# LiWentomng/OrientedRepPoints

Measured on NVIDIA H100. Metric: 1024x1024 tiles/sec, higher is better.
Workload: dtype f16x3

## Files before the change

include/orp_b200.h:

```cpp
#ifndef ORP_B200_H_
#define ORP_B200_H_

#include <stdint.h>

#ifdef __cplusplus
extern "C" {
#endif

#define ORP_OK 0
#define ORP_EINVAL (-1)
#define ORP_ECUDA (-2)
#define ORP_ENOGPU (-3)
#define ORP_EOVERFLOW (-4)

const char *orp_last_error(void);
int orp_version(void);
int orp_compiled_sm(void);
int64_t orp_launch_count(void);
void orp_reset_launch_count(void);


#define ORP_NMS_EXACT64 0
#define ORP_NMS_COMPAT32 1

#define ORP_UNION_NAN_KEEPS 0
#define ORP_UNION_GUARD 1
#define ORP_UNION_NAN_SUPPRESSES 2
#define ORP_UNION_NAN_SUPPRESSES_ALL 3

#define ORP_ORDER_INDEX_ASC 0
#define ORP_ORDER_SCORE_DESC 1

int orp_rnms(const float *dets, const int32_t *segments, int n, double iou_thr, int iou_mode,
             int union_mode, int order, int64_t *keep_out, int32_t *num_out, void *stream);

int orp_poly_nms_host(int *keep_out, int *num_out, const float *polys_host, int polys_num,
                      int polys_dim, float nms_overlap_thresh, int device_id);

typedef struct {
    int64_t pairs_total;
    int64_t pairs_aabb;
    int64_t pairs_clipped;
    int64_t pairs_fp64;
    int64_t edges;
    int64_t suppressing;
    int32_t overflow;
    int32_t rounds;
    int32_t n;
} orp_nms_stats;
int orp_rnms_last_stats(orp_nms_stats *out);

typedef struct {
    int32_t lazy;
    int32_t R;
    int32_t seg_limit;
    int32_t sweep_bits;
    int32_t no_sync;
    int32_t flags_out;
    int32_t union_mode, order, n;
    int64_t cap_first;
    int64_t cap_final;
    int32_t attempts;
} orp_rnms_plan;
int orp_rnms_last_plan(orp_rnms_plan *out);

void orp_set_timing(int on);
int orp_rnms_last_sweep_ms(float *ms);
int orp_tc_timing_collect(float *total_ms, int *launches, double *flops);
typedef struct {
    int BN;
    int stages;
    int grid;
    int num_tiles;
    int n_tiles_n;
    int ksplit;
    int nprob;
    int Cout, Cout_padded;
    int split;
    int deform;
    int out_f32;
    int stem;
    int relu;
    int bias;
    int residual;
    int tma_epi, ncat, dcat, res_mma, b_resident, epi_merge, epi_bufs, gn_fused;
    int BW[5], BH[5], BI[5];
    int n_pair;
} orp_tc_plan;
int orp_tc_last_plan(orp_tc_plan *out);


int orp_poly_overlaps_host(float *overlaps, const float *boxes, const float *query_boxes, int n,
                           int k, int device_id);
int orp_poly_overlaps(const float *boxes5, int n, const float *query5, int k, float *out,
                      void *stream);

int orp_quad_iou_matrix(const float *quads_a, int n, const float *quads_b, int k, int iou_mode,
                        int union_mode, float *out, void *stream);

int orp_iou_poly_f64_pairs(const double *p8, const double *q8, int n, double *out, void *stream);

int orp_convex_iou(const float *pts18, int n, const float *quads8, int k, float *out, void *stream);

int orp_box_iou_rotated(const float *boxes1, int n, const float *boxes2, int m, float *out,
                        void *stream);


int orp_minarearect(const float *pts, int n, float *out, int32_t *hull_map, float scale,
                    const float *center, void *stream);


int orp_head_postprocess(int nlevels, const float *const *cls, const float *const *ref, const int *H,
                         const int *W, const int *stride, int B, int num_cls, int nms_pre, float score_thr,
                         double iou_thr, int max_per_img, const float *scale_factor, float *dets_out,
                         int64_t *labels_out, int32_t *counts_out, void *stream);
int orp_head_postprocess_aug(int nviews, int nlevels, const float *const *cls, const float *const *ref, const int *H,
                             const int *W, const int *stride, int B, int num_cls, int nms_pre, float score_thr,
                             double iou_thr, int max_per_img, const float *view_meta, const float *out_scale,
                             float *dets_out, int64_t *labels_out, int32_t *counts_out, void *stream);
int orp_pack_detections(const float *dets, const int64_t *labels, const int32_t *counts, int B, int max_per_img,
                        float *packed_out, void *stream);
int orp_dcn_offsets_multi(int nprob, const float *const *pts, float *const *off, const long long *numel,
                          float gradient_mul, const float *base18, void *stream);


#define ORP_MERGE_BAD_COUNT 1
#define ORP_MERGE_BAD_TILE 2
#define ORP_MERGE_ROWS_OVERFLOW 4

int orp_result_merge(const float *packed, int S, int cap, const int32_t *tile_slot, const int32_t *tile_xy,
                     const double *tile_rate, const int32_t *tile_img, int Tn, int ncls, int nimg, double thresh,
                     int union_mode, int max_rows, int32_t *count_out, int64_t *cls_off_out, int32_t *cls_out,
                     int32_t *img_out, double *score_out, double *quad_out, int32_t *src_row_out, int32_t *status_out,
                     void *stream);


int orp_dota_eval_task1(const int32_t *det_cls, const int32_t *det_img, const double *det_score, const double *det_quad,
                        int nd, const int32_t *gt_cls, const int32_t *gt_img, const double *gt_quad,
                        const uint8_t *gt_difficult, int ng, int ncls, int nimg, double ovthresh, int use_07_metric,
                        const double *thresholds11, int64_t *npos_out, int64_t *cls_off_out, int32_t *order_out,
                        double *rec_out, double *prec_out, double *ap_out, void *stream);

int orp_poly2rbox_v3(const double *quad, int n, double *out, void *stream);

int orp_dota_eval_aoe(const int32_t *det_cls, const int32_t *det_img, const double *det_score, const double *det_quad,
                      int nd, const int32_t *gt_cls, const int32_t *gt_img, const double *gt_quad, int ng, int ncls,
                      int nimg, double ovthresh, int64_t *cls_off_out, int32_t *order_out, double *angle_dif_out,
                      int64_t *count_out, double *aoe_out, void *stream);


int orp_convex_giou(const float *pts18, const float *quads8, int n, float *out19, void *stream);


int orp_conv2d_f32(const float *x, int N, int H, int W, int Cin, const float *w, int Cout, int KH, int KW,
                   int stride, int pad, const float *bias, const float *residual, int relu, float *y,
                   double *gn_stats, int groups, void *stream);

int orp_deform_conv2d_f32(const float *x, int N, int H, int W, int Cin, const float *offset, const float *mask,
                          const float *w, int Cout, int KH, int KW, int stride, int pad, int dilation,
                          const float *bias, int relu, float *y, void *stream);

int orp_gn_apply_f32(const float *x, int N, int H, int W, int C, const double *stats, int groups,
                     const float *gamma, const float *beta, float eps, int relu, const float *up_src, float *y,
                     void *stream);

int orp_maxpool3x3s2_f32(const float *x, int N, int H, int W, int C, float *y, void *stream);


typedef struct {
    const void *x;
    int N, H, W;
    void *out;
    const void *residual_bf16;
    const float *residual_f32;
    const float *offset;
    double *gn_stats;
    const float *mask;
} orp_tc_problem;

int orp_conv2d_bf16(int nprob, const orp_tc_problem *probs, const void *w, int Cout, int Cout_padded,
                    int KH, int KW, int Cin, int stride, int pad, const float *bias, int relu, int out_f32,
                    int deform, void *stream);

int orp_conv2d_f16x3(int nprob, const orp_tc_problem *probs, const void *w_split, int Cout, int Cout_padded,
                     int KH, int KW, int Cin, int stride, int pad, const float *bias, int wscale_log2, int relu,
                     int out_f32, int deform, void *stream);
int orp_conv2d_tc_splitk(const orp_tc_problem *prob, const void *w, int Cout, int Cout_padded, int KH, int KW, int Cin,
                         int stride, int pad, const float *bias, int f16x3, int wscale_log2, int relu, int ksplit,
                         float *workspace, void *stream);
int orp_tc_plan_conv(int nprob, const orp_tc_problem *probs, const void *w, int Cout, int Cout_padded, int KH, int KW,
                     int Cin, int stride, int pad, const float *bias, int wscale_log2, int relu, int out_f32, int deform,
                     int split, int stem, int ksplit, int sms, orp_tc_plan *out);
int orp_f16x3_overflow_count(unsigned int *count, int reset, void *stream);
int orp_stem_s2d_u8_f16x3(const uint8_t *img_hwc, int N, int H, int W, const float *mean, const float *std, int to_rgb,
                          void *out, void *stream);
int orp_stem_s2d_u8_padded_f16x3(const uint8_t *img_hwc, int N, int H, int W, const float *mean, const float *std, int to_rgb,
                                 const int32_t *valid_hw, void *out, void *stream);
int orp_stem_s2d_f16x3(const float *img_nchw, int N, int H, int W, void *out, void *stream);
int orp_stem_conv_s2d_f16x3(const void *x_s2d, int N, int H, int W, const void *w_split, const float *bias,
                            int wscale_log2, int relu, void *out, void *stream);
int orp_maxpool3x3s2_f16x3(const void *x, int N, int H, int W, int C, void *y, void *stream);
int orp_gn_stats_f16x3(const void *x, int N, int HW, int C, int groups, double *stats, void *stream);
int orp_split_from_f32(const float *x, long long pixels, int C, void *y_split, void *stream);
int orp_split_to_f32(const void *x_split, long long pixels, int C, float *y, void *stream);
int orp_transpose_f32(const float *x, int N, int R, int Cc, float *y, void *stream);
int orp_nchw_f32_to_split(const float *x, int N, int C, int HW, void *y_split, void *stream);

int orp_stem_im2col_bf16(const float *img_nchw, int N, int H, int W, void *out, void *stream);
int orp_stem_s2d_bf16(const float *img_nchw, int N, int H, int W, void *out, void *stream);
int orp_stem_conv_s2d_bf16(const void *x_s2d, int N, int H, int W, const void *w256, const float *bias, int relu,
                           void *out, void *stream);
int orp_stem_s2d_u8_bf16(const uint8_t *img_hwc, int N, int H, int W, const float *mean, const float *std, int to_rgb,
                         void *out, void *stream);
int orp_stem_s2d_u8_padded_bf16(const uint8_t *img_hwc, int N, int H, int W, const float *mean, const float *std, int to_rgb,
                                const int32_t *valid_hw, void *out, void *stream);
int orp_maxpool3x3s2_bf16(const void *x, int N, int H, int W, int C, void *y, void *stream);
int orp_gn_stats_bf16(const void *x, int N, int HW, int C, int groups, double *stats, void *stream);
typedef struct orp_gn_problem {
    const void *x;
    int N, H, W;
    const double *stats;
    const void *up_src;
    void *y;
} orp_gn_problem;
int orp_gn_apply_bf16_multi(int nprob, const orp_gn_problem *probs, int C, int groups, const float *gamma,
                            const float *beta, float eps, int relu, void *stream);
int orp_gn_apply_f16x3_multi(int nprob, const orp_gn_problem *probs, int C, int groups, const float *gamma,
                             const float *beta, float eps, int relu, void *stream);

int orp_split_tiles_u8(const uint8_t *img_hwc, int H, int W, int C, const int32_t *origins, int ntiles, int subsize,
                       uint8_t *out, void *stream);

int orp_resize_u8(const uint8_t *src, int N, int H, int W, int C, uint8_t *dst, int Hd, int Wd, int Hp, int Wp, int flip,
                  const int32_t *xtab, const int32_t *ytab, void *stream);


int orp_layernorm_bf16(const void *x, int B, int H, int W, int C, const float *gamma, const float *beta, float eps,
                       int Hp, int Wp, void *y, void *stream);
int orp_window_attention_bf16(const void *qkv, int B, int H, int W, int Hp, int Wp, int C, int heads, int shift,
                              const float *bias_table, float scale, void *out, void *stream);
int orp_patch_embed_rows_bf16(const float *img_nchw, int B, int H, int W, void *out, void *stream);
int orp_patch_embed_rows_u8_bf16(const uint8_t *img_hwc, int B, int H, int W, const float *mean, const float *stdinv, int to_rgb,
                                 void *out, void *stream);
int orp_patch_embed_rows_u8_padded_bf16(const uint8_t *img_hwc, int B, int H, int W, const float *mean, const float *stdinv,
                                        int to_rgb, const int32_t *valid_hw, void *out, void *stream);
int orp_patch_merge_gather_bf16(const void *x, int B, int H, int W, int C, void *y, void *stream);
int orp_subsample2_bf16(const void *x, int B, int H, int W, int C, void *y, void *stream);
int orp_layernorm_f16x3(const void *x, int B, int H, int W, int C, const float *gamma, const float *beta, float eps,
                        int Hp, int Wp, void *y, void *stream);
int orp_window_attention_f16x3(const void *qkv, int B, int H, int W, int Hp, int Wp, int C, int heads, int shift,
                               const float *bias_table, float scale, void *out, void *stream);
int orp_patch_embed_rows_f16x3(const float *img_nchw, int B, int H, int W, void *out, void *stream);
int orp_patch_embed_rows_u8_f16x3(const uint8_t *img_hwc, int B, int H, int W, const float *mean, const float *stdinv, int to_rgb,
                                  void *out, void *stream);
int orp_patch_embed_rows_u8_padded_f16x3(const uint8_t *img_hwc, int B, int H, int W, const float *mean, const float *stdinv,
                                         int to_rgb, const int32_t *valid_hw, void *out, void *stream);
int orp_patch_merge_gather_f16x3(const void *x, int B, int H, int W, int C, void *y, void *stream);
int orp_subsample2_f16x3(const void *x, int B, int H, int W, int C, void *y, void *stream);

#ifdef __cplusplus
}
#endif
#endif
```

orientedreppoints_b200/_lib.py:

```python
import ctypes
import os

_HERE = os.path.dirname(os.path.abspath(__file__))
LIB_PATH = os.path.join(_HERE, "lib", "liborp_b200.so")

ORP_NMS_EXACT64, ORP_NMS_COMPAT32 = 0, 1
ORP_UNION_NAN_KEEPS, ORP_UNION_GUARD, ORP_UNION_NAN_SUPPRESSES, ORP_UNION_NAN_SUPPRESSES_ALL = 0, 1, 2, 3
ORP_ORDER_INDEX_ASC, ORP_ORDER_SCORE_DESC = 0, 1
ORP_MERGE_BAD_COUNT, ORP_MERGE_BAD_TILE, ORP_MERGE_ROWS_OVERFLOW = 1, 2, 4

_vp = ctypes.c_void_p
_i = ctypes.c_int
_f = ctypes.c_float
_d = ctypes.c_double


class NmsStats(ctypes.Structure):
    _fields_ = [("pairs_total", ctypes.c_int64), ("pairs_aabb", ctypes.c_int64),
                ("pairs_clipped", ctypes.c_int64), ("pairs_fp64", ctypes.c_int64),
                ("edges", ctypes.c_int64), ("suppressing", ctypes.c_int64), ("overflow", ctypes.c_int32),
                ("rounds", ctypes.c_int32), ("n", ctypes.c_int32)]

    def as_dict(self):
        return {k: int(getattr(self, k)) for k, _ in self._fields_}


class RnmsPlan(ctypes.Structure):
    _fields_ = [(k, ctypes.c_int32) for k in ("lazy", "R", "seg_limit", "sweep_bits", "no_sync", "flags_out", "union_mode",
                                              "order", "n")] + \
              [("cap_first", ctypes.c_int64), ("cap_final", ctypes.c_int64), ("attempts", ctypes.c_int32)]

    def as_dict(self):
        return {k: int(getattr(self, k)) for k, _ in self._fields_}


class TcProblem(ctypes.Structure):
    _fields_ = [("x", _vp), ("N", _i), ("H", _i), ("W", _i), ("out", _vp), ("residual_bf16", _vp),
                ("residual_f32", _vp), ("offset", _vp), ("gn_stats", _vp), ("mask", _vp)]


class TcPlan(ctypes.Structure):
    _fields_ = [(k, _i) for k in ("BN", "stages", "grid", "num_tiles", "n_tiles_n", "ksplit", "nprob", "Cout", "Cout_padded",
                                  "split", "deform", "out_f32", "stem", "relu", "bias", "residual", "tma_epi", "ncat", "dcat",
                                  "res_mma", "b_resident", "epi_merge", "epi_bufs", "gn_fused")] + \
              [(k, _i * 5) for k in ("BW", "BH", "BI")] + [("n_pair", _i)]

    def as_dict(self):
        d = {k: getattr(self, k) for k, _ in self._fields_}
        for k in ("BW", "BH", "BI"):
            d[k] = list(d[k])[:self.nprob]
        return d


class GnProblem(ctypes.Structure):
    _fields_ = [("x", _vp), ("N", _i), ("H", _i), ("W", _i), ("stats", _vp), ("up_src", _vp), ("y", _vp)]


SIGNATURES = {
    "orp_last_error": (ctypes.c_char_p, []),
    "orp_version": (_i, []),
    "orp_compiled_sm": (_i, []),
    "orp_launch_count": (ctypes.c_int64, []),
    "orp_reset_launch_count": (None, []),
    "orp_rnms": (_i, [_vp, _vp, _i, _d, _i, _i, _i, _vp, _vp, _vp]),
    "orp_poly_nms_host": (_i, [_vp, _vp, _vp, _i, _i, _f, _i]),
    "orp_rnms_last_stats": (_i, [ctypes.POINTER(NmsStats)]),
    "orp_rnms_last_plan": (_i, [ctypes.POINTER(RnmsPlan)]),
    "orp_set_timing": (None, [_i]),
    "orp_rnms_last_sweep_ms": (_i, [ctypes.POINTER(ctypes.c_float)]),
    "orp_tc_timing_collect": (_i, [ctypes.POINTER(ctypes.c_float), ctypes.POINTER(_i), ctypes.POINTER(_d)]),
    "orp_tc_last_plan": (_i, [ctypes.POINTER(TcPlan)]),
    "orp_poly_overlaps_host": (_i, [_vp, _vp, _vp, _i, _i, _i]),
    "orp_poly_overlaps": (_i, [_vp, _i, _vp, _i, _vp, _vp]),
    "orp_quad_iou_matrix": (_i, [_vp, _i, _vp, _i, _i, _i, _vp, _vp]),
    "orp_iou_poly_f64_pairs": (_i, [_vp, _vp, _i, _vp, _vp]),
    "orp_box_iou_rotated": (_i, [_vp, _i, _vp, _i, _vp, _vp]),
    "orp_minarearect": (_i, [_vp, _i, _vp, _vp, _f, _vp, _vp]),
    "orp_head_postprocess": (_i, [_i, _vp, _vp, _vp, _vp, _vp, _i, _i, _i, _f, _d, _i, _vp, _vp, _vp, _vp, _vp]),
    "orp_head_postprocess_aug": (_i, [_i, _i, _vp, _vp, _vp, _vp, _vp, _i, _i, _i, _f, _d, _i, _vp, _vp, _vp, _vp, _vp, _vp]),
    "orp_pack_detections": (_i, [_vp, _vp, _vp, _i, _i, _vp, _vp]),
    "orp_dcn_offsets_multi": (_i, [_i, _vp, _vp, _vp, _f, _vp, _vp]),
    "orp_conv2d_f32": (_i, [_vp, _i, _i, _i, _i, _vp, _i, _i, _i, _i, _i, _vp, _vp, _i, _vp, _vp, _i, _vp]),
    "orp_deform_conv2d_f32": (_i, [_vp, _i, _i, _i, _i, _vp, _vp, _vp, _i, _i, _i, _i, _i, _i, _vp, _i, _vp, _vp]),
    "orp_gn_apply_f32": (_i, [_vp, _i, _i, _i, _i, _vp, _i, _vp, _vp, _f, _i, _vp, _vp, _vp]),
    "orp_maxpool3x3s2_f32": (_i, [_vp, _i, _i, _i, _i, _vp, _vp]),
    "orp_conv2d_bf16": (_i, [_i, ctypes.POINTER(TcProblem), _vp, _i, _i, _i, _i, _i, _i, _i, _vp, _i, _i, _i, _vp]),
    "orp_conv2d_f16x3": (_i, [_i, ctypes.POINTER(TcProblem), _vp, _i, _i, _i, _i, _i, _i, _i, _vp, _i, _i, _i, _i, _vp]),
    "orp_conv2d_tc_splitk": (_i, [ctypes.POINTER(TcProblem), _vp, _i, _i, _i, _i, _i, _i, _i, _vp, _i, _i, _i, _i, _vp, _vp]),
    "orp_tc_plan_conv": (_i, [_i, ctypes.POINTER(TcProblem), _vp, _i, _i, _i, _i, _i, _i, _i, _vp, _i, _i, _i, _i, _i, _i, _i, _i,
                              ctypes.POINTER(TcPlan)]),
    "orp_f16x3_overflow_count": (_i, [ctypes.POINTER(ctypes.c_uint), _i, _vp]),
    "orp_stem_s2d_u8_f16x3": (_i, [_vp, _i, _i, _i, _vp, _vp, _i, _vp, _vp]),
    "orp_stem_s2d_f16x3": (_i, [_vp, _i, _i, _i, _vp, _vp]),
    "orp_stem_conv_s2d_f16x3": (_i, [_vp, _i, _i, _i, _vp, _vp, _i, _i, _vp, _vp]),
    "orp_maxpool3x3s2_f16x3": (_i, [_vp, _i, _i, _i, _i, _vp, _vp]),
    "orp_gn_stats_f16x3": (_i, [_vp, _i, _i, _i, _i, _vp, _vp]),
    "orp_gn_apply_f16x3_multi": (_i, [_i, _vp, _i, _i, _vp, _vp, _f, _i, _vp]),
    "orp_split_from_f32": (_i, [_vp, ctypes.c_longlong, _i, _vp, _vp]),
    "orp_split_to_f32": (_i, [_vp, ctypes.c_longlong, _i, _vp, _vp]),
    "orp_transpose_f32": (_i, [_vp, _i, _i, _i, _vp, _vp]),
    "orp_nchw_f32_to_split": (_i, [_vp, _i, _i, _i, _vp, _vp]),
    "orp_layernorm_bf16": (_i, [_vp, _i, _i, _i, _i, _vp, _vp, _f, _i, _i, _vp, _vp]),
    "orp_window_attention_bf16": (_i, [_vp, _i, _i, _i, _i, _i, _i, _i, _i, _vp, _f, _vp, _vp]),
    "orp_patch_embed_rows_bf16": (_i, [_vp, _i, _i, _i, _vp, _vp]),
    "orp_patch_embed_rows_u8_bf16": (_i, [_vp, _i, _i, _i, _vp, _vp, _i, _vp, _vp]),
    "orp_patch_merge_gather_bf16": (_i, [_vp, _i, _i, _i, _i, _vp, _vp]),
    "orp_subsample2_bf16": (_i, [_vp, _i, _i, _i, _i, _vp, _vp]),
    "orp_layernorm_f16x3": (_i, [_vp, _i, _i, _i, _i, _vp, _vp, _f, _i, _i, _vp, _vp]),
    "orp_window_attention_f16x3": (_i, [_vp, _i, _i, _i, _i, _i, _i, _i, _i, _vp, _f, _vp, _vp]),
    "orp_patch_embed_rows_f16x3": (_i, [_vp, _i, _i, _i, _vp, _vp]),
    "orp_patch_embed_rows_u8_f16x3": (_i, [_vp, _i, _i, _i, _vp, _vp, _i, _vp, _vp]),
    "orp_patch_merge_gather_f16x3": (_i, [_vp, _i, _i, _i, _i, _vp, _vp]),
    "orp_subsample2_f16x3": (_i, [_vp, _i, _i, _i, _i, _vp, _vp]),
    "orp_stem_im2col_bf16": (_i, [_vp, _i, _i, _i, _vp, _vp]),
    "orp_stem_s2d_bf16": (_i, [_vp, _i, _i, _i, _vp, _vp]),
    "orp_convex_iou": (_i, [_vp, _i, _vp, _i, _vp, _vp]),
    "orp_convex_giou": (_i, [_vp, _vp, _i, _vp, _vp]),
    "orp_dota_eval_task1": (_i, [_vp, _vp, _vp, _vp, _i, _vp, _vp, _vp, _vp, _i, _i, _i, _d, _i, _vp, _vp, _vp, _vp, _vp,
                                 _vp, _vp, _vp]),
    "orp_dota_eval_aoe": (_i, [_vp, _vp, _vp, _vp, _i, _vp, _vp, _vp, _i, _i, _i, _d, _vp, _vp, _vp, _vp, _vp, _vp]),
    "orp_poly2rbox_v3": (_i, [_vp, _i, _vp, _vp]),
    "orp_result_merge": (_i, [_vp, _i, _i, _vp, _vp, _vp, _vp, _i, _i, _i, _d, _i, _i, _vp, _vp, _vp, _vp, _vp, _vp, _vp, _vp,
                              _vp]),
    "orp_split_tiles_u8": (_i, [_vp, _i, _i, _i, _vp, _i, _i, _vp, _vp]),
    "orp_resize_u8": (_i, [_vp, _i, _i, _i, _i, _vp, _i, _i, _i, _i, _i, _vp, _vp, _vp]),
    "orp_stem_s2d_u8_padded_bf16": (_i, [_vp, _i, _i, _i, _vp, _vp, _i, _vp, _vp, _vp]),
    "orp_stem_s2d_u8_padded_f16x3": (_i, [_vp, _i, _i, _i, _vp, _vp, _i, _vp, _vp, _vp]),
    "orp_patch_embed_rows_u8_padded_bf16": (_i, [_vp, _i, _i, _i, _vp, _vp, _i, _vp, _vp, _vp]),
    "orp_patch_embed_rows_u8_padded_f16x3": (_i, [_vp, _i, _i, _i, _vp, _vp, _i, _vp, _vp, _vp]),
    "orp_stem_s2d_u8_bf16": (_i, [_vp, _i, _i, _i, _vp, _vp, _i, _vp, _vp]),
    "orp_stem_conv_s2d_bf16": (_i, [_vp, _i, _i, _i, _vp, _vp, _i, _vp, _vp]),
    "orp_maxpool3x3s2_bf16": (_i, [_vp, _i, _i, _i, _i, _vp, _vp]),
    "orp_gn_stats_bf16": (_i, [_vp, _i, _i, _i, _i, _vp, _vp]),
    "orp_gn_apply_bf16_multi": (_i, [_i, _vp, _i, _i, _vp, _vp, _f, _i, _vp]),
}

_LIB = None


class OrpError(RuntimeError):
    pass


def lib():
    global _LIB
    if _LIB is None:
        if not os.path.exists(LIB_PATH):
            raise OrpError(
                "liborp_b200.so not found at %s - build it with `python -m orientedreppoints_b200.build` "
                "(there is no CPU or PyTorch fallback for this path)" % LIB_PATH)
        l = ctypes.CDLL(LIB_PATH)
        for name, (res, args) in SIGNATURES.items():
            fn = getattr(l, name)
            fn.restype = res
            fn.argtypes = args
        _LIB = l
    return _LIB


def check(rc, what=""):
    if rc != 0:
        msg = lib().orp_last_error()
        raise OrpError("%s failed (%d): %s" % (what, rc, msg.decode() if msg else ""))


def launch_count():
    return int(lib().orp_launch_count())


def reset_launch_count():
    lib().orp_reset_launch_count()


def last_nms_stats():
    s = NmsStats()
    check(lib().orp_rnms_last_stats(ctypes.byref(s)), "orp_rnms_last_stats")
    return s.as_dict()


def rnms_last_plan():
    p = RnmsPlan()
    check(lib().orp_rnms_last_plan(ctypes.byref(p)), "orp_rnms_last_plan")
    return p.as_dict()


def set_timing(on):
    lib().orp_set_timing(1 if on else 0)


def last_sweep_ms():
    v = ctypes.c_float(0)
    check(lib().orp_rnms_last_sweep_ms(ctypes.byref(v)), "orp_rnms_last_sweep_ms")
    return float(v.value)


def tc_timing_collect():
    ms, n, fl = ctypes.c_float(0), ctypes.c_int(0), ctypes.c_double(0)
    check(lib().orp_tc_timing_collect(ctypes.byref(ms), ctypes.byref(n), ctypes.byref(fl)), "orp_tc_timing_collect")
    return float(ms.value), int(n.value), float(fl.value)


def tc_last_plan():
    p = TcPlan()
    check(lib().orp_tc_last_plan(ctypes.byref(p)), "orp_tc_last_plan")
    return p.as_dict()


def tc_plan_for(problems, cout, cout_p, kh, kw, cin, stride, pad, *, bias=False, relu=0, out_f32=False, deform=False,
                split=False, residual=0, gn=False, stem=0, ksplit=1, sms=132):
    ph = 256
    arr = (TcProblem * len(problems))()
    for q, (n, h, w) in zip(arr, problems):
        q.x, q.N, q.H, q.W, q.out = ph, n, h, w, ph
        q.residual_bf16 = ph if residual == 1 else None
        q.residual_f32 = ph if residual == 2 else None
        q.offset = ph if deform else None
        q.gn_stats = ph if gn else None
    p = TcPlan()
    check(lib().orp_tc_plan_conv(len(problems), arr, ph, cout, cout_p, kh, kw, cin, stride, pad, ph if bias else None, 0,
                                 int(relu), int(out_f32), int(deform), int(split), stem, ksplit, sms, ctypes.byref(p)),
          "orp_tc_plan_conv")
    return p.as_dict()


def current_stream_ptr():
    import torch
    return ctypes.c_void_p(torch.cuda.current_stream().cuda_stream)


def ptr(t):
    return ctypes.c_void_p(0 if t is None else t.data_ptr())
```

orientedreppoints_b200/csrc/dense_tc.cu:

```cuda
#include <cuda.h>
#include <cuda_bf16.h>
#include <cuda_fp16.h>

#include <cstdlib>
#include <mutex>
#include <type_traits>

#include "common.cuh"
#include "wgmma.cuh"

namespace orp {
namespace {

constexpr int kMaxProb = 5;
constexpr int kStagesMax = 6;
constexpr int kBM = 128;
constexpr int kBK = 64;
constexpr int kABytes = kBM * kBK * 2;

struct FastDiv {
    uint32_t mul, shr, d;
    __host__ void set(uint32_t div)
    {
        d = div;
        uint32_t l = 0;
        while ((1ull << l) < div) ++l;
        shr = l;
        mul = (uint32_t)(((1ull << 32) * ((1ull << l) - div)) / div + 1);
    }
    __device__ __forceinline__ uint32_t div(uint32_t n) const { return (__umulhi(n, mul) + n) >> shr; }
    __device__ __forceinline__ void divmod(uint32_t n, uint32_t &q, uint32_t &r) const { q = div(n); r = n - q * d; }
};

struct Problem {
    int N, H, W, Ho, Wo;
    FastDiv fd_tw, fd_th;
    int BW, BH, BI;
    int lbw, lbh;
    int tiles_w, tiles_h, tiles_i, tile_start;
    void *out;
    const __nv_bfloat16 *res;
    const float *res32;
    const __nv_bfloat16 *x;
    const float *offset;
    const float *mask;
    double *gn_stats;
};

struct alignas(64) TcParams {
    CUtensorMap tmA[kMaxProb];
    CUtensorMap tmB;
    CUtensorMap tmOut[kMaxProb];
    CUtensorMap tmRes[kMaxProb];
    CUtensorMap tmI;
    Problem prob[kMaxProb];
    int tma_epi, epi_bufs;
    int epi_merge;
    int ncat;
    int ksplit;
    FastDiv fd_ks;
    long long ks_stride;
    int b_resident;
    int res_mma;
    int gn_fused;
    int dcat;
    int split;
    float oscale;
    unsigned int *ovf;
    int nprob, num_m_tiles, n_tiles_n, num_tiles;
    FastDiv fd_ntn;
    int KH, KW, Cin, cin_blocks, stride, pad, Cout, relu;
    int s2d_stem;
    const float *bias;
};

__device__ __forceinline__ uint32_t smem_u32(const void *p) { return (uint32_t)__cvta_generic_to_shared(p); }

__device__ __forceinline__ void mbar_init(uint64_t *bar, uint32_t count)
{
    asm volatile("mbarrier.init.shared::cta.b64 [%0], %1;" ::"r"(smem_u32(bar)), "r"(count));
}
__device__ __forceinline__ void mbar_expect_tx(uint64_t *bar, uint32_t bytes)
{
    asm volatile("mbarrier.arrive.expect_tx.shared::cta.b64 _, [%0], %1;" ::"r"(smem_u32(bar)), "r"(bytes) : "memory");
}
__device__ __forceinline__ void mbar_arrive(uint64_t *bar)
{
    asm volatile("mbarrier.arrive.shared::cta.b64 _, [%0];" ::"r"(smem_u32(bar)) : "memory");
}
__device__ __forceinline__ void mbar_wait(uint64_t *bar, uint32_t parity)
{
    asm volatile(
        "{\n\t"
        ".reg .pred p;\n\t"
        "WAIT_LOOP:\n\t"
        "mbarrier.try_wait.parity.shared::cta.b64 p, [%0], %1;\n\t"
        "@p bra WAIT_DONE;\n\t"
        "bra WAIT_LOOP;\n\t"
        "WAIT_DONE:\n\t"
        "}" ::"r"(smem_u32(bar)), "r"(parity) : "memory");
}
__device__ __forceinline__ bool elect_one()
{
    uint32_t pred = 0;
    asm volatile(
        "{\n\t"
        ".reg .pred P1;\n\t"
        "elect.sync _|P1, %1;\n\t"
        "selp.b32 %0, 1, 0, P1;\n\t"
        "}" : "=r"(pred) : "r"(0xffffffffu));
    return pred != 0;
}
__device__ __forceinline__ void tma_load_4d(void *smem, const CUtensorMap *tm, uint64_t *bar, int c0, int c1, int c2, int c3)
{
    asm volatile(
        "cp.async.bulk.tensor.4d.shared::cluster.global.mbarrier::complete_tx::bytes [%0], [%1, {%3, %4, %5, %6}], [%2];"
        ::"r"(smem_u32(smem)), "l"(tm), "r"(smem_u32(bar)), "r"(c0), "r"(c1), "r"(c2), "r"(c3) : "memory");
}
__device__ __forceinline__ void tma_load_5d(void *smem, const CUtensorMap *tm, uint64_t *bar, int c0, int c1, int c2, int c3, int c4)
{
    asm volatile(
        "cp.async.bulk.tensor.5d.shared::cluster.global.mbarrier::complete_tx::bytes [%0], [%1, {%3, %4, %5, %6, %7}], [%2];"
        ::"r"(smem_u32(smem)), "l"(tm), "r"(smem_u32(bar)), "r"(c0), "r"(c1), "r"(c2), "r"(c3), "r"(c4) : "memory");
}
__device__ __forceinline__ void tma_load_2d(void *smem, const CUtensorMap *tm, uint64_t *bar, int c0, int c1)
{
    asm volatile(
        "cp.async.bulk.tensor.2d.shared::cluster.global.mbarrier::complete_tx::bytes [%0], [%1, {%3, %4}], [%2];"
        ::"r"(smem_u32(smem)), "l"(tm), "r"(smem_u32(bar)), "r"(c0), "r"(c1) : "memory");
}
__device__ __forceinline__ uint64_t make_desc_sw128(uint32_t smem_addr)
{
    uint64_t d = 0;
    d |= (uint64_t)((smem_addr >> 4) & 0x3FFF);
    d |= (uint64_t)1 << 16;
    d |= (uint64_t)(1024 >> 4) << 32;
    d |= (uint64_t)1 << 62;
    return d;
}
__device__ __forceinline__ uint4 lds128(uint32_t addr)
{
    uint4 v;
    asm volatile("ld.shared.v4.b32 {%0, %1, %2, %3}, [%4];" : "=r"(v.x), "=r"(v.y), "=r"(v.z), "=r"(v.w) : "r"(addr) : "memory");
    return v;
}
__device__ __forceinline__ void sts128(uint32_t addr, const uint4 &v)
{
    asm volatile("st.shared.v4.b32 [%0], {%1, %2, %3, %4};" ::"r"(addr), "r"(v.x), "r"(v.y), "r"(v.z), "r"(v.w) : "memory");
}
template <int ID, int N>
__device__ __forceinline__ void named_bar()
{
    asm volatile("bar.sync %0, %1;" ::"n"(ID), "n"(N) : "memory");
}
__device__ __forceinline__ void acc_ld32(uint32_t addr, uint32_t (&r)[32])
{
#pragma unroll
    for (int j = 0; j < 8; ++j) {
        const uint4 v = lds128(addr + (uint32_t)j * 16u);
        r[4 * j] = v.x; r[4 * j + 1] = v.y; r[4 * j + 2] = v.z; r[4 * j + 3] = v.w;
    }
}

__device__ __forceinline__ float2 ffma2_rn(float2 a, float2 b, float2 c) { return make_float2(__fmaf_rn(a.x, b.x, c.x), __fmaf_rn(a.y, b.y, c.y)); }
__device__ __forceinline__ float2 fadd2_rn(float2 a, float2 b) { return make_float2(__fadd_rn(a.x, b.x), __fadd_rn(a.y, b.y)); }

__device__ __forceinline__ void split_sample(const uint4 (&u)[4][2], float4 wv, uint2 wh, uint32_t (&hi)[4], uint32_t (&lo)[4])
{
    const float2 wc[4] = {make_float2(wv.x, wv.x), make_float2(wv.y, wv.y), make_float2(wv.z, wv.z), make_float2(wv.w, wv.w)};
    const __half2 wl[4] = {__low2half2(*reinterpret_cast<const __half2 *>(&wh.x)), __high2half2(*reinterpret_cast<const __half2 *>(&wh.x)),
                           __low2half2(*reinterpret_cast<const __half2 *>(&wh.y)), __high2half2(*reinterpret_cast<const __half2 *>(&wh.y))};
#pragma unroll
    for (int k = 0; k < 4; ++k) {
        float2 acc = make_float2(0.f, 0.f);
        __half2 accl = __float2half2_rn(0.f);
#pragma unroll
        for (int c = 0; c < 4; ++c) {
            const uint32_t uh = reinterpret_cast<const uint32_t *>(&u[c][0])[k];
            const uint32_t ul = reinterpret_cast<const uint32_t *>(&u[c][1])[k];
            acc = ffma2_rn(wc[c], __half22float2(*reinterpret_cast<const __half2 *>(&uh)), acc);
            accl = __hfma2(wl[c], *reinterpret_cast<const __half2 *>(&ul), accl);
        }
        acc = fadd2_rn(acc, __half22float2(accl));
        const __half2 h2 = __floats2half2_rn(acc.x, acc.y);
        const float2 hf = __half22float2(h2);
        const float2 rem = fadd2_rn(acc, make_float2(-hf.x, -hf.y));
        const __half2 l2 = __floats2half2_rn(rem.x, rem.y);
        hi[k] = *reinterpret_cast<const uint32_t *>(&h2);
        lo[k] = *reinterpret_cast<const uint32_t *>(&l2);
    }
}

__device__ __forceinline__ float act_fn(float v, int act)
{
    if (act == 1) return fmaxf(v, 0.f);
    if (act == 2) return 0.5f * v * (1.0f + erff(v * 0.70710678118654752f));
    return v;
}

struct Ring {
    int stage = 0;
    uint32_t phase = 0;
    int n;
    __device__ explicit Ring(int n_) : n(n_) {}
    __device__ void next() { if (++stage == n) { stage = 0; phase ^= 1; } }
};

struct KIter {
    int tap, term, cb = 0, phase = 0;
    int tap0, taps, cbn, mode;
    __device__ KIter(int taps_, int cbn_, int mode_, int tap0_ = 0) : tap0(tap0_), taps(taps_), cbn(cbn_), mode(mode_)
    {
        tap = tap0;
        term = (mode == 1) ? 1 : 0;
    }
    __device__ void next()
    {
        if (mode == 0) { if (++cb == cbn) { cb = 0; ++tap; } }
        else if (phase == 0) {
            if (++cb == cbn) { cb = 0; if (++term == 3) { term = 1; if (++tap == taps) { tap = tap0; term = 0; phase = 1; } } }
        } else { if (++cb == cbn) { cb = 0; ++tap; } }
    }
};

__device__ __forceinline__ int ksplit_of(const TcParams &P, int tile)
{
    if (P.ksplit <= 1) return 0;
    uint32_t q, r;
    P.fd_ks.divmod((uint32_t)tile, q, r);
    return (int)r;
}

__device__ __forceinline__ void decode_tile(const TcParams &P, int tile, int &pi, int &wb, int &hb, int &ib, int &nt)
{
    uint32_t mt_u, nt_u;
    if (P.ksplit > 1) tile = (int)P.fd_ks.div((uint32_t)tile);
    P.fd_ntn.divmod((uint32_t)tile, mt_u, nt_u);
    nt = (int)nt_u;
    const int mt = (int)mt_u;
    pi = 0;
#pragma unroll
    for (int k = 1; k < kMaxProb; ++k)
        if (k < P.nprob && mt >= P.prob[k].tile_start) pi = k;
    const Problem &pr = P.prob[pi];
    const int local = mt - pr.tile_start;
    uint32_t rest, wb_u, ib_u, hb_u;
    pr.fd_tw.divmod((uint32_t)local, rest, wb_u);
    pr.fd_th.divmod(rest, ib_u, hb_u);
    wb = (int)wb_u; hb = (int)hb_u; ib = (int)ib_u;
}

struct IdentBlock { unsigned short v[64 * 64]; };
constexpr IdentBlock make_ident()
{
    IdentBlock b{};
    for (int i = 0; i < 64; ++i) b.v[i * 64 + i] = 0x3F80;
    return b;
}
__device__ IdentBlock g_ident = make_ident();
struct IdentBlocks16 { unsigned short v[16][64 * 64]; };
constexpr IdentBlocks16 make_ident16()
{
    IdentBlocks16 b{};
    for (int s = 0; s < 16; ++s)
        for (int i = 0; i < 64; ++i) b.v[s][i * 64 + i] = (unsigned short)((15 + s) << 10);
    return b;
}
__device__ IdentBlocks16 g_ident16 = make_ident16();
__device__ unsigned int g_f16_overflow = 0;

constexpr int kConsumers = 256;
constexpr int kDP = 256;
constexpr int kDItems = 1024 / kDP;
constexpr int kDRound = kDItems / 2;
constexpr int kAccPitch = 68;
constexpr int kAccBytes = 128 * kAccPitch * 4;

__host__ __device__ constexpr int stage_bytes(int BN, bool cat, bool b_resident)
{
    return cat ? (b_resident ? 2 * kABytes : 2 * kABytes + 2 * BN * kBK * 2) : (b_resident ? kABytes : kABytes + BN * kBK * 2);
}
__host__ __device__ constexpr bool frag_epilogue(int BN, bool deform) { return deform && BN == 256; }
constexpr int dyn_smem_bytes(int stage_b, int stages, int extra, bool frag_epi)
{
    return 1024 + (frag_epi ? 0 : kAccBytes) + stages * stage_b + extra;
}

template <int BN, int R>
__device__ __forceinline__ void stage_acc(const float (&acc)[R], int pass, bool ncat, float *s_acc, int row0, int col0)
{
    constexpr int kGroups = (BN < 64 ? BN : 64) / 8;
#pragma unroll
    for (int p = 0; p < (BN + 63) / 64; ++p) {
        if (p != pass) continue;
#pragma unroll
        for (int i = 0; i < kGroups; ++i) {
            const int g = p * 8 + i;
            float2 a = make_float2(acc[4 * g], acc[4 * g + 1]), b = make_float2(acc[4 * g + 2], acc[4 * g + 3]);
            if constexpr (R >= BN) {
                if (ncat) {
                    a.x += acc[BN / 2 + 4 * g]; a.y += acc[BN / 2 + 4 * g + 1];
                    b.x += acc[BN / 2 + 4 * g + 2]; b.y += acc[BN / 2 + 4 * g + 3];
                }
            }
            *reinterpret_cast<float2 *>(s_acc + row0 * kAccPitch + i * 8 + col0) = a;
            *reinterpret_cast<float2 *>(s_acc + (row0 + 8) * kAccPitch + i * 8 + col0) = b;
        }
    }
}

constexpr int kWalkK = 0;
constexpr int kWalkNcat = 1;
constexpr int kWalkDcat = 2;
constexpr int kWalkKRes = 3;

template <int NG, bool BF16, int R, int G = 0>
__device__ __forceinline__ void wgmma_cols64(float (&acc)[R], uint64_t da, uint64_t db, uint32_t accumulate)
{
    wgmma_n<64, BF16>(acc_view<32 * G, 32>(acc), da, db + (uint64_t)(G * 512), accumulate);
    if constexpr (G + 1 < NG) wgmma_cols64<NG, BF16, R, G + 1>(acc, da, db, accumulate);
}

template <int BN, bool BF16>
__device__ __forceinline__ void wgmma_dcat(float (&acc)[BN / 2], uint64_t da, uint64_t db, uint32_t accumulate)
{
    if constexpr (BN == 256) {
        wgmma_n<128, BF16>(acc_view<0, 64>(acc), da, db, accumulate);
        wgmma_n<128, BF16>(acc_view<64, 64>(acc), da, db + (uint64_t)1024, accumulate);
    } else {
        wgmma_n<BN, BF16>(acc, da, db, accumulate);
    }
}

constexpr int kProducerRegs = 40;
constexpr int kConsumerRegs = 232;
constexpr int kWideConsumerRegs = 160;
constexpr int kWideProducerRegs = 96;

template <int BN, bool OUT_F32, bool DEFORM, bool SPLIT, int WALK>
__global__ void __launch_bounds__(DEFORM ? kConsumers + kDP : kConsumers + 128, 1)
conv_tc_kernel(const __grid_constant__ TcParams P, int stages)
{
    static_assert(WALK != kWalkNcat || (SPLIT && !DEFORM && !OUT_F32 && BN >= 64 && BN <= 128), "ncat: f16x3 TMA-epilogue layers, BN 64..128");
    static_assert(!DEFORM || (WALK == kWalkDcat) == SPLIT, "deformable: dcat exactly in f16x3");
    static_assert(DEFORM || WALK != kWalkDcat, "dcat is the deformable walk");
    static_assert(WALK != kWalkKRes || (!DEFORM && !OUT_F32 && BN >= 64), "residual K blocks: TMA-epilogue layers");
    constexpr bool kBF16 = !SPLIT;
    constexpr int kWTerms = SPLIT ? 2 : 1;
    constexpr bool kCat = WALK == kWalkNcat || WALK == kWalkDcat;
    constexpr int kKMode = (SPLIT && !kCat) ? 1 : 0;
    static_assert(kConsumers + 128 == 384 && 2 * 128 * kConsumerRegs + 128 * kProducerRegs <= 65536, "register split");
    constexpr bool kFragEpi = frag_epilogue(BN, DEFORM);
    static_assert(!kFragEpi || (SPLIT && !OUT_F32), "fragment epilogue: deformable f16x3 with a TMA epilogue");
    static_assert(kConsumers == 256 && kDP == 256 && 2 * 128 * kWideConsumerRegs + 2 * 128 * kWideProducerRegs <= 65536,
                  "register split (wide deformable)");
    constexpr int kEpiThreads = kConsumers;
    constexpr int kWG = 2;
    constexpr int kAccN = (WALK == kWalkNcat) ? 2 * BN : BN;
    extern __shared__ __align__(1024) uint8_t smem_raw[];
    uint8_t *smem = reinterpret_cast<uint8_t *>((reinterpret_cast<uintptr_t>(smem_raw) + 1023) & ~uintptr_t(1023));
    float *s_acc = reinterpret_cast<float *>(smem);
    if constexpr (!kFragEpi) smem += kAccBytes;
    constexpr int kBBytes = BN * kBK * 2;
    const int kStageBytes = stage_bytes(BN, kCat, P.b_resident);
    const int kblocks_all = P.KH * P.KW * P.cin_blocks * kWTerms;
    uint8_t *ident = smem;
    if (P.res_mma) smem += 8192;
    uint8_t *bres = smem;
    if (P.b_resident) smem += (size_t)kblocks_all * kBBytes;
    constexpr int HC = BN < 64 ? BN : 64;
    constexpr int kPitch = HC * 2 + 16;
    uint8_t *stage_out = smem + (size_t)stages * kStageBytes;
    __shared__ uint64_t bars[2 * kStagesMax];
    __shared__ __align__(16) float s_bias[256];
    __shared__ uint64_t bres_bar;
    uint64_t *full = bars;
    uint64_t *empty = bars + kStagesMax;

    const int warp = threadIdx.x >> 5, lane = threadIdx.x & 31;

    if (warp == kConsumers / 32 && elect_one()) {
        if (!DEFORM) {
#pragma unroll 1
            for (int p = 0; p < P.nprob; ++p)
                asm volatile("prefetch.tensormap [%0];" ::"l"(&P.tmA[p]) : "memory");
        }
        asm volatile("prefetch.tensormap [%0];" ::"l"(&P.tmB) : "memory");
    }
    if (warp == 0) {
        if (elect_one()) {
            for (int s = 0; s < stages; ++s) {
                mbar_init(&full[s], DEFORM ? 1 + kDP / 32 : 1);
                mbar_init(&empty[s], kConsumers / 128);
            }
            mbar_init(&bres_bar, 1);
            asm volatile("fence.mbarrier_init.release.cluster;" ::: "memory");
        }
        __syncwarp();
    }
    __syncthreads();
    const int taps_per = (P.KH * P.KW) / (P.ksplit > 1 ? P.ksplit : 1);
    const int kblocks = taps_per * P.cin_blocks * (kKMode ? 3 : 1);
    asm volatile("griddepcontrol.launch_dependents;" ::: "memory");
    asm volatile("griddepcontrol.wait;" ::: "memory");

    if (warp < kConsumers / 32) {
        if constexpr (!DEFORM) setmaxnreg_inc<kConsumerRegs>();
        if constexpr (kFragEpi) setmaxnreg_inc<kWideConsumerRegs>();
        const int cw = warp >> 2;
        const uint32_t a_off = (uint32_t)cw * 8192u;
        const bool leader = (threadIdx.x & 127) == 0;
        float acc[kAccN / 2];
        Ring r(stages);
        const int q = warp & 3, wg = warp >> 2;
        const int et = threadIdx.x, nthr = kEpiThreads;
        const int bar_a = 1, bar_b = 3;
        const int ch0 = wg, chs = kWG;
        const int frow = cw * 64 + (warp & 3) * 16 + (lane >> 2), fcol = 2 * (lane & 3);
        const uint32_t s_acc_u = smem_u32(s_acc);
        auto bar_sync = [](int id, int n) { asm volatile("bar.sync %0, %1;" ::"r"(id), "r"(n) : "memory"); };
        int ob = 0;
        int bias_nt = -1;
        if ((P.b_resident || P.res_mma) && (int)blockIdx.x < P.num_tiles) mbar_wait(&bres_bar, 0);
        for (int tile = blockIdx.x; tile < P.num_tiles; tile += gridDim.x) {
            int res_groups = 0;
            if constexpr (WALK == kWalkKRes) {
                const int nt = tile - (int)P.fd_ntn.div((uint32_t)tile) * P.n_tiles_n;
                for (int g = 0; g < BN / 64 && nt * BN + g * 64 < P.Cout; ++g) ++res_groups;
            }
            const int tap_lo = ksplit_of(P, tile) * taps_per;
            KIter it(tap_lo + taps_per, P.cin_blocks, kKMode, tap_lo);
            int held = -1;
            auto release = [&](int next) {
                if (held >= 0 && leader) mbar_arrive(&empty[held]);
                held = next;
            };
            for (int kb = 0; kb < kblocks; ++kb, it.next()) {
                if constexpr (kFragEpi) {
                    wgmma_wait<0>();
                    release(-1);
                }
                mbar_wait(&full[r.stage], r.phase);
                const uint32_t sa = smem_u32(smem + (size_t)r.stage * kStageBytes);
                const uint64_t da = make_desc_sw128(sa + a_off);
                const int slab = (it.tap * P.cin_blocks + it.cb) * kWTerms + (it.term == 2 ? 1 : 0);
                wgmma_fence();
                if constexpr (WALK == kWalkNcat) {
                    const uint32_t sb = P.b_resident ? smem_u32(bres + (size_t)slab * kBBytes) : sa + 2 * kABytes;
                    const uint64_t dl = make_desc_sw128(sa + kABytes + a_off);
                    const uint64_t dbh = make_desc_sw128(sb), dbl = make_desc_sw128(sb + kBBytes);
#pragma unroll
                    for (int k = 0; k < kBK / 16; ++k) {
                        const uint32_t first = (kb | k) ? 1u : 0u;
                        wgmma_n<BN, kBF16>(acc_view<0, BN / 2>(acc), da + (uint64_t)(k * 2), dbh + (uint64_t)(k * 2), first);
                        wgmma_n<BN, kBF16>(acc_view<BN / 2, BN / 2>(acc), da + (uint64_t)(k * 2), dbl + (uint64_t)(k * 2), first);
                        wgmma_n<BN, kBF16>(acc_view<BN / 2, BN / 2>(acc), dl + (uint64_t)(k * 2), dbh + (uint64_t)(k * 2), 1u);
                    }
                } else if constexpr (WALK == kWalkDcat) {
                    const uint64_t dl = make_desc_sw128(sa + kABytes + a_off);
                    const uint64_t dbh = make_desc_sw128(sa + 2 * kABytes), dbl = make_desc_sw128(sa + 2 * kABytes + kBBytes);
#pragma unroll
                    for (int k = 0; k < kBK / 16; ++k) {
                        wgmma_dcat<BN, kBF16>(acc, dl + (uint64_t)(k * 2), dbh + (uint64_t)(k * 2), (kb | k) ? 1u : 0u);
                        wgmma_dcat<BN, kBF16>(acc, da + (uint64_t)(k * 2), dbl + (uint64_t)(k * 2), 1u);
                        wgmma_dcat<BN, kBF16>(acc, da + (uint64_t)(k * 2), dbh + (uint64_t)(k * 2), 1u);
                    }
                } else {
                    const uint64_t db = make_desc_sw128(P.b_resident ? smem_u32(bres + (size_t)slab * kBBytes) : sa + kABytes);
#pragma unroll
                    for (int k = 0; k < kBK / 16; ++k) {
                        if constexpr (WALK == kWalkKRes)
                            wgmma_cols64<BN / 64, kBF16>(acc, da + (uint64_t)(k * 2), db + (uint64_t)(k * 2), (kb | k) ? 1u : 0u);
                        else
                            wgmma_n<BN, kBF16>(acc, da + (uint64_t)(k * 2), db + (uint64_t)(k * 2), (kb | k) ? 1u : 0u);
                    }
                }
                wgmma_commit();
                wgmma_wait<1>();
                release(r.stage);
                r.next();
            }
            if constexpr (WALK == kWalkKRes) {
                wgmma_wait<0>();
                release(-1);
                auto res_group = [&](auto gc) {
                    constexpr int G = decltype(gc)::value;
                    if (G >= res_groups) return;
#pragma unroll 1
                    for (int t = 0; t < kWTerms; ++t) {
                        mbar_wait(&full[r.stage], r.phase);
                        const uint64_t da = make_desc_sw128(smem_u32(smem + (size_t)r.stage * kStageBytes) + a_off);
                        const uint64_t db = make_desc_sw128(smem_u32(ident));
                        wgmma_fence();
#pragma unroll
                        for (int k = 0; k < kBK / 16; ++k)
                            wgmma_n<64, kBF16>(acc_view<32 * G, 32>(acc), da + (uint64_t)(k * 2), db + (uint64_t)(k * 2), 1u);
                        wgmma_commit();
                        wgmma_wait<1>();
                        release(r.stage);
                        r.next();
                    }
                };
                res_group(std::integral_constant<int, 0>{});
                if constexpr (BN >= 128) res_group(std::integral_constant<int, 1>{});
                if constexpr (BN >= 256) {
                    res_group(std::integral_constant<int, 2>{});
                    res_group(std::integral_constant<int, 3>{});
                }
            }
            wgmma_wait<0>();
            wgmma_fence_acc(acc);
            release(-1);

            int pi, wb, hb, ib, nt;
            decode_tile(P, tile, pi, wb, hb, ib, nt);
            const Problem &pr = P.prob[pi];
            const int rrow = q * 32 + lane;
            auto row_pixel = [&](int r, size_t &pix) -> bool {
                const int iw = r & (pr.BW - 1), ih = (r >> pr.lbw) & (pr.BH - 1), ii = r >> (pr.lbw + pr.lbh);
                const int w = wb * pr.BW + iw, h = hb * pr.BH + ih, n = ib * pr.BI + ii;
                pix = ((size_t)n * pr.Ho + h) * pr.Wo + w;
                return (w < pr.Wo) && (h < pr.Ho) && (n < pr.N);
            };
            size_t pix;
            const bool valid = row_pixel(rrow, pix);
            if constexpr (kFragEpi) {
                const uint32_t obuf_u = smem_u32(stage_out);
                const bool io = (et == 0);
                if (nt != bias_nt) {
                    bar_sync(bar_a, nthr);
                    for (int c = et; c < BN; c += nthr) s_bias[c] = (P.bias && nt * BN + c < P.Cout) ? P.bias[nt * BN + c] : 0.f;
                    bias_nt = nt;
                }
                size_t pix_r[2];
                const bool valid_r[2] = {row_pixel(frow, pix_r[0]), row_pixel(frow + 8, pix_r[1])};
                float amax[2][2] = {{0.f, 0.f}, {0.f, 0.f}};
#pragma unroll
                for (int pass = 0; pass < 2 * (BN / 64); ++pass) {
                    const int half = pass >> 1, oterm = pass & 1;
                    if (io) {
                        if (P.epi_bufs == 2) asm volatile("cp.async.bulk.wait_group.read 1;" ::: "memory");
                        else asm volatile("cp.async.bulk.wait_group.read 0;" ::: "memory");
                    }
                    bar_sync(bar_a, nthr);
                    const uint32_t obase = obuf_u + (uint32_t)ob * 16384u;
#pragma unroll
                    for (int i = 0; i < 8; ++i) {
                        const int g = half * 8 + i;
                        const float2 bv = *reinterpret_cast<const float2 *>(&s_bias[g * 8 + fcol]);
#pragma unroll
                        for (int hr = 0; hr < 2; ++hr) {
                            const int row = frow + 8 * hr;
                            float f0 = acc[4 * g + 2 * hr], f1 = acc[4 * g + 2 * hr + 1];
                            f0 *= P.oscale; f1 *= P.oscale;
                            f0 += bv.x; f1 += bv.y;
                            if (P.relu) { f0 = fmaxf(f0, 0.f); f1 = fmaxf(f1, 0.f); }
                            if (oterm == 0) amax[hr][i >> 2] = fmaxf(fmaxf(amax[hr][i >> 2], fabsf(f0)), fabsf(f1));
                            const __half2 h2 = __floats2half2_rn(f0, f1);
                            uint32_t v = *reinterpret_cast<const uint32_t *>(&h2);
                            if (oterm) {
                                const float2 hf = __half22float2(h2);
                                const __half2 l2 = __floats2half2_rn(f0 - hf.x, f1 - hf.y);
                                v = *reinterpret_cast<const uint32_t *>(&l2);
                            }
                            const uint32_t at = obase + (uint32_t)row * 128u + ((uint32_t)(i ^ (row & 7)) << 4) + (uint32_t)fcol * 2u;
                            asm volatile("st.shared.b32 [%0], %1;" ::"r"(at), "r"(v) : "memory");
                        }
                    }
                    asm volatile("fence.proxy.async.shared::cta;" ::: "memory");
                    bar_sync(bar_b, nthr);
                    if (io) {
                        asm volatile(
                            "cp.async.bulk.tensor.5d.global.shared::cta.bulk_group [%0, {%2, %3, %4, %5, %6}], [%1];"
                            ::"l"(&P.tmOut[pi]), "r"(obase), "r"(nt * BN + half * 64), "r"(oterm),
                              "r"(wb * pr.BW), "r"(hb * pr.BH), "r"(ib * pr.BI) : "memory");
                        asm volatile("cp.async.bulk.commit_group;" ::: "memory");
                    }
                    if (++ob == P.epi_bufs) ob = 0;
                }
#pragma unroll
                for (int hr = 0; hr < 2; ++hr)
#pragma unroll
                    for (int hc = 0; hc < 2; ++hc) {
                        float m = amax[hr][hc];
                        m = fmaxf(m, __shfl_xor_sync(0xffffffffu, m, 1));
                        m = fmaxf(m, __shfl_xor_sync(0xffffffffu, m, 2));
                        if ((lane & 3) == 0 && valid_r[hr] && m > 65504.f) atomicAdd(P.ovf, 1u);
                    }
            } else if (OUT_F32) {
#pragma unroll 1
                for (int pass = 0; pass < BN / HC; ++pass) {
                bar_sync(bar_a, nthr);
                stage_acc<BN>(acc, pass, false, s_acc, frow, fcol);
                bar_sync(bar_a, nthr);
#pragma unroll 1
                for (int ch = wg; ch < HC / 32; ch += kWG) {
                    uint32_t v[32];
                    acc_ld32(s_acc_u + (uint32_t)(rrow * kAccPitch + ch * 32) * 4u, v);
                    const int c0 = nt * BN + pass * HC + ch * 32;
                    if (valid && c0 < P.Cout) {
                        float *op = reinterpret_cast<float *>(pr.out) + pix * P.Cout + c0;
                        const float *rp = pr.res32 ? pr.res32 + pix * P.Cout + c0 : nullptr;
                        if (P.ksplit > 1) {
                            float *sp = op + (long long)ksplit_of(P, tile) * P.ks_stride;
                            for (int j = 0; j < 32; ++j) {
                                if (c0 + j >= P.Cout) break;
                                sp[j] = __uint_as_float(v[j]) * P.oscale;
                            }
                        } else
                        for (int j = 0; j < 32; ++j) {
                            if (c0 + j >= P.Cout) break;
                            float f = __uint_as_float(v[j]) * P.oscale;
                            if (P.bias) f += P.bias[c0 + j];
                            if (pr.res && !P.split) f += __bfloat162float(pr.res[pix * P.Cout + c0 + j]);
                            if (rp) f += rp[j];
                            f = act_fn(f, P.relu);
                            op[j] = f;
                        }
                    }
                }
                }
            } else if (P.tma_epi) {
                const uint32_t slot = P.epi_merge ? 32768u : 16384u;
                const uint32_t obuf_u = smem_u32(stage_out);
                const uint32_t bias_u = smem_u32(s_bias);
                const bool io = (et == 0);
                constexpr int kPasses = BN / 64;
                const int oterms = (P.split && !P.epi_merge) ? 2 : 1;
                if (nt != bias_nt) {
                    bar_sync(bar_a, nthr);
                    for (int c = et; c < BN; c += nthr) s_bias[c] = (P.bias && nt * BN + c < P.Cout) ? P.bias[nt * BN + c] : 0.f;
                    bias_nt = nt;
                }
                float amax = 0.f;
#pragma unroll 1
                for (int pass = 0; pass < kPasses * oterms; ++pass) {
                    const int half = oterms == 2 ? (pass >> 1) : pass, oterm = oterms == 2 ? (pass & 1) : 0;
                    if (io) {
                        if (P.epi_bufs == 2) asm volatile("cp.async.bulk.wait_group.read 1;" ::: "memory");
                        else asm volatile("cp.async.bulk.wait_group.read 0;" ::: "memory");
                    }
                    bar_sync(bar_a, nthr);
                    if (oterm == 0) {
                        stage_acc<BN>(acc, half, P.ncat != 0, s_acc, frow, fcol);
                        bar_sync(bar_a, nthr);
                    }
                    float gn_s = 0.f, gn_q = 0.f;
                    const uint32_t orow = obuf_u + (uint32_t)ob * slot + (uint32_t)rrow * 128u;
#pragma unroll 1
                    for (int ch = ch0; ch < 2; ch += chs) {
                        const uint32_t arow = s_acc_u + (uint32_t)(rrow * kAccPitch + ch * 32) * 4u;
#pragma unroll
                        for (int j4 = 0; j4 < 4; ++j4) {
                            const int c16 = ch * 4 + j4;
                            const uint32_t sw = (uint32_t)(c16 ^ (rrow & 7)) << 4;
                            const uint4 a0 = lds128(arow + (uint32_t)j4 * 32u), a1 = lds128(arow + (uint32_t)j4 * 32u + 16u);
                            const float f0[8] = {__uint_as_float(a0.x), __uint_as_float(a0.y), __uint_as_float(a0.z), __uint_as_float(a0.w),
                                                 __uint_as_float(a1.x), __uint_as_float(a1.y), __uint_as_float(a1.z), __uint_as_float(a1.w)};
                            float f[8];
#pragma unroll
                            for (int j = 0; j < 8; ++j) f[j] = f0[j];
                            const uint32_t bb = bias_u + (uint32_t)(half * 64 + ch * 32 + j4 * 8) * 4u;
                            const uint4 b0 = lds128(bb), b1 = lds128(bb + 16u);
                            if (P.split) {
#pragma unroll
                                for (int j = 0; j < 8; ++j) f[j] *= P.oscale;
                            }
                            f[0] += __uint_as_float(b0.x); f[1] += __uint_as_float(b0.y);
                            f[2] += __uint_as_float(b0.z); f[3] += __uint_as_float(b0.w);
                            f[4] += __uint_as_float(b1.x); f[5] += __uint_as_float(b1.y);
                            f[6] += __uint_as_float(b1.z); f[7] += __uint_as_float(b1.w);
                            if (P.relu == 2) {
#pragma unroll
                                for (int j = 0; j < 8; ++j) f[j] = act_fn(f[j], 2);
                            }
                            uint32_t pk[4];
                            if (P.split) {
#pragma unroll
                                for (int j = 0; j < 8; ++j) {
                                    if (P.relu == 1) f[j] = fmaxf(f[j], 0.f);
                                    if (oterm == 0) amax = fmaxf(amax, fabsf(f[j]));
                                }
                                uint32_t pl[4];
#pragma unroll
                                for (int k = 0; k < 4; ++k) {
                                    const __half2 h2 = __floats2half2_rn(f[2 * k], f[2 * k + 1]);
                                    pk[k] = *reinterpret_cast<const uint32_t *>(&h2);
                                    if (P.epi_merge || oterm) {
                                        const float2 hf = __half22float2(h2);
                                        const __half2 l2 = __floats2half2_rn(f[2 * k] - hf.x, f[2 * k + 1] - hf.y);
                                        pl[k] = *reinterpret_cast<const uint32_t *>(&l2);
                                    }
                                }
                                if (P.epi_merge) sts128(orow + 16384u + sw, make_uint4(pl[0], pl[1], pl[2], pl[3]));
                                else if (oterm) { pk[0] = pl[0]; pk[1] = pl[1]; pk[2] = pl[2]; pk[3] = pl[3]; }
                            } else {
#pragma unroll
                                for (int k = 0; k < 4; ++k) {
                                    __nv_bfloat162 b2 = __floats2bfloat162_rn(f[2 * k], f[2 * k + 1]);
                                    if (P.relu == 1) b2 = __hmax2(b2, __floats2bfloat162_rn(0.f, 0.f));
                                    pk[k] = *reinterpret_cast<uint32_t *>(&b2);
                                }
                            }
                            sts128(orow + sw, make_uint4(pk[0], pk[1], pk[2], pk[3]));
                            if (P.gn_fused && oterm == 0) {
                                float gs = 0.f, gq = 0.f;
                                if (valid) {
#pragma unroll
                                    for (int j = 0; j < 8; ++j) { gs += f[j]; gq = fmaf(f[j], f[j], gq); }
                                }
#pragma unroll
                                for (int o = 16; o > 0; o >>= 1) {
                                    gs += __shfl_xor_sync(0xffffffffu, gs, o);
                                    gq += __shfl_xor_sync(0xffffffffu, gq, o);
                                }
                                if (lane == c16) { gn_s = gs; gn_q = gq; }
                            }
                        }
                    }
                    if (P.gn_fused && oterm == 0 && lane < 8 && (chs == 1 || (lane >> 2) == wg)) {
                        const int n_img = ib * pr.BI + ((q * 32) >> (pr.lbw + pr.lbh));
                        if (n_img < pr.N) {
                            double *st = pr.gn_stats + ((size_t)n_img * 32 + (size_t)(nt * BN + half * 64) / 8 + lane) * 2;
                            atomicAdd(st, (double)gn_s);
                            atomicAdd(st + 1, (double)gn_q);
                        }
                    }
                    asm volatile("fence.proxy.async.shared::cta;" ::: "memory");
                    bar_sync(bar_b, nthr);
                    if (io) {
                        asm volatile(
                            "cp.async.bulk.tensor.5d.global.shared::cta.bulk_group [%0, {%2, %3, %4, %5, %6}], [%1];"
                            ::"l"(&P.tmOut[pi]), "r"(obuf_u + (uint32_t)ob * slot), "r"(nt * BN + half * 64), "r"(oterm),
                              "r"(wb * pr.BW), "r"(hb * pr.BH), "r"(ib * pr.BI) : "memory");
                        if (P.epi_merge)
                            asm volatile(
                                "cp.async.bulk.tensor.5d.global.shared::cta.bulk_group [%0, {%2, %3, %4, %5, %6}], [%1];"
                                ::"l"(&P.tmOut[pi]), "r"(obuf_u + (uint32_t)ob * slot + 16384u), "r"(nt * BN + half * 64), "r"(1),
                                  "r"(wb * pr.BW), "r"(hb * pr.BH), "r"(ib * pr.BI) : "memory");
                        asm volatile("cp.async.bulk.commit_group;" ::: "memory");
                    }
                    if (++ob == P.epi_bufs) ob = 0;
                }
                if (P.split && valid && amax > 65504.f) atomicAdd(P.ovf, 1u);
            } else {
                const bool vec_ok = (P.Cout & 7) == 0;
                named_bar<1, kEpiThreads>();
                for (int c = et; c < BN; c += kEpiThreads) s_bias[c] = (P.bias && nt * BN + c < P.Cout) ? P.bias[nt * BN + c] : 0.f;
                named_bar<1, kEpiThreads>();
#pragma unroll 1
                for (int half = 0; half < BN / HC; ++half) {
                    const int cbase = nt * BN + half * HC;
                    constexpr int kChunksPerRow = HC / 8;
                    if (pr.res && vec_ok) {
                        for (int c = et; c < 128 * kChunksPerRow; c += kEpiThreads) {
                            const int r = c / kChunksPerRow, k16 = c - r * kChunksPerRow;
                            size_t rp;
                            const bool ok = row_pixel(r, rp) && (cbase + k16 * 8 < P.Cout);
                            const uint32_t dst = smem_u32(stage_out + (size_t)r * kPitch + k16 * 16);
                            if (ok) {
                                const __nv_bfloat16 *src = pr.res + rp * P.Cout + cbase + k16 * 8;
                                asm volatile("cp.async.cg.shared.global [%0], [%1], 16;" ::"r"(dst), "l"(src) : "memory");
                            }
                        }
                        asm volatile("cp.async.commit_group;" ::: "memory");
                    }
                    if (pr.res && vec_ok) asm volatile("cp.async.wait_group 0;" ::: "memory");
                    stage_acc<BN>(acc, half, false, s_acc, frow, fcol);
                    named_bar<1, kEpiThreads>();
#pragma unroll 1
                    for (int ch = wg; ch < HC / 32; ch += kWG) {
                        uint32_t v[32];
                        acc_ld32(s_acc_u + (uint32_t)(rrow * kAccPitch + ch * 32) * 4u, v);
                        const int c0 = cbase + ch * 32;
                        uint4 *sp = reinterpret_cast<uint4 *>(stage_out + (size_t)rrow * kPitch + ch * 64);
#pragma unroll
                        for (int j4 = 0; j4 < 4; ++j4) {
                            float f[8];
#pragma unroll
                            for (int j = 0; j < 8; ++j) f[j] = __uint_as_float(v[j4 * 8 + j]);
                            {
                                const float4 b0 = *reinterpret_cast<const float4 *>(&s_bias[half * HC + ch * 32 + j4 * 8]);
                                const float4 b1 = *reinterpret_cast<const float4 *>(&s_bias[half * HC + ch * 32 + j4 * 8 + 4]);
                                f[0] += b0.x; f[1] += b0.y; f[2] += b0.z; f[3] += b0.w;
                                f[4] += b1.x; f[5] += b1.y; f[6] += b1.z; f[7] += b1.w;
                            }
                            if (pr.res && !vec_ok && valid) {
                                for (int j = 0; j < 8; ++j)
                                    if (c0 + j4 * 8 + j < P.Cout) f[j] += __bfloat162float(pr.res[pix * P.Cout + c0 + j4 * 8 + j]);
                            }
                            if (pr.res && vec_ok && valid) {
                                const uint4 u = sp[j4];
                                const uint32_t uu[4] = {u.x, u.y, u.z, u.w};
#pragma unroll
                                for (int k = 0; k < 4; ++k) {
                                    const float2 r2 = __bfloat1622float2(*reinterpret_cast<const __nv_bfloat162 *>(&uu[k]));
                                    f[2 * k] += r2.x;
                                    f[2 * k + 1] += r2.y;
                                }
                            }
                            if (P.relu) {
#pragma unroll
                                for (int j = 0; j < 8; ++j) f[j] = act_fn(f[j], P.relu);
                            }
                            uint32_t pk[4];
#pragma unroll
                            for (int k = 0; k < 4; ++k) {
                                __nv_bfloat162 b2 = __floats2bfloat162_rn(f[2 * k], f[2 * k + 1]);
                                pk[k] = *reinterpret_cast<uint32_t *>(&b2);
                            }
                            sp[j4] = make_uint4(pk[0], pk[1], pk[2], pk[3]);
                        }
                    }
                    named_bar<1, kEpiThreads>();
                    for (int c = et; c < 128 * kChunksPerRow; c += kEpiThreads) {
                        const int r = c / kChunksPerRow, k16 = c - r * kChunksPerRow;
                        size_t rp;
                        if (row_pixel(r, rp) && (cbase + k16 * 8 < P.Cout)) {
                            const uint4 u = *reinterpret_cast<const uint4 *>(stage_out + (size_t)r * kPitch + k16 * 16);
                            __nv_bfloat16 *op = reinterpret_cast<__nv_bfloat16 *>(pr.out) + rp * P.Cout + cbase + k16 * 8;
                            if (vec_ok) {
                                *reinterpret_cast<uint4 *>(op) = u;
                            } else {
                                const __nv_bfloat16 *e8 = reinterpret_cast<const __nv_bfloat16 *>(&u);
                                for (int j = 0; j < 8; ++j) if (cbase + k16 * 8 + j < P.Cout) op[j] = e8[j];
                            }
                        }
                    }
                    named_bar<1, kEpiThreads>();
                }
            }
        }
        if (P.tma_epi && et == 0) asm volatile("cp.async.bulk.wait_group 0;" ::: "memory");
    } else if (!DEFORM) {
        setmaxnreg_dec<kProducerRegs>();
        if (warp == kConsumers / 32 && elect_one()) {
            Ring r(stages);
            if ((P.b_resident || P.res_mma) && (int)blockIdx.x < P.num_tiles) {
                const int nt0 = blockIdx.x % P.n_tiles_n;
                mbar_expect_tx(&bres_bar, (uint32_t)((P.b_resident ? kblocks_all * kBBytes : 0) + (P.res_mma ? 8192 : 0)));
                if (P.res_mma) tma_load_2d(ident, &P.tmI, &bres_bar, 0, 0);
                if (P.b_resident)
                    for (int kb = 0; kb < kblocks_all; ++kb)
                        tma_load_2d(bres + (size_t)kb * kBBytes, &P.tmB, &bres_bar, kb * kBK, nt0 * BN);
            }
            for (int tile = blockIdx.x; tile < P.num_tiles; tile += gridDim.x) {
                int pi, wb, hb, ib, nt;
                decode_tile(P, tile, pi, wb, hb, ib, nt);
                const Problem &pr = P.prob[pi];
                const int w0 = wb * pr.BW * P.stride - P.pad, h0 = hb * pr.BH * P.stride - P.pad, i0 = ib * pr.BI;
                const int tap_lo = ksplit_of(P, tile) * taps_per;
                KIter it(tap_lo + taps_per, P.cin_blocks, kKMode, tap_lo);
                for (int j = 0; j < kblocks; ++j, it.next()) {
                    const int kh = it.tap / P.KW, kw = it.tap - kh * P.KW;
                    mbar_wait(&empty[r.stage], r.phase ^ 1);
                    uint8_t *sa = smem + (size_t)r.stage * kStageBytes;
                    const int wblk = ((it.tap * P.cin_blocks + it.cb) * kWTerms) * kBK;
                    if constexpr (WALK == kWalkNcat) {
                        mbar_expect_tx(&full[r.stage], 2 * kABytes + (P.b_resident ? 0 : 2 * kBBytes));
                        tma_load_5d(sa, &P.tmA[pi], &full[r.stage], it.cb * kBK, 0, w0 + kw, h0 + kh, i0);
                        tma_load_5d(sa + kABytes, &P.tmA[pi], &full[r.stage], it.cb * kBK, 1, w0 + kw, h0 + kh, i0);
                        if (!P.b_resident) {
                            tma_load_2d(sa + 2 * kABytes, &P.tmB, &full[r.stage], wblk, nt * BN);
                            tma_load_2d(sa + 2 * kABytes + kBBytes, &P.tmB, &full[r.stage], wblk + kBK, nt * BN);
                        }
                    } else {
                        mbar_expect_tx(&full[r.stage], P.b_resident ? kABytes : kABytes + kBBytes);
                        tma_load_5d(sa, &P.tmA[pi], &full[r.stage], it.cb * kBK, it.term == 1 ? 1 : 0, w0 + kw, h0 + kh, i0);
                        if (!P.b_resident)
                            tma_load_2d(sa + kABytes, &P.tmB, &full[r.stage], wblk + (it.term == 2 ? kBK : 0), nt * BN);
                    }
                    r.next();
                }
                if constexpr (WALK == kWalkKRes) {
                    for (int g = 0; g < BN / 64 && nt * BN + g * 64 < P.Cout; ++g)
                        for (int t = 0; t < kWTerms; ++t) {
                            mbar_wait(&empty[r.stage], r.phase ^ 1);
                            mbar_expect_tx(&full[r.stage], kABytes);
                            tma_load_5d(smem + (size_t)r.stage * kStageBytes, &P.tmRes[pi], &full[r.stage], nt * BN + g * 64, t,
                                        wb * pr.BW, hb * pr.BH, ib * pr.BI);
                            r.next();
                        }
                }
            }
        }
    } else if (DEFORM) {
        __shared__ float4 s_w[2][128];
        __shared__ uint2 s_wh[2][128];
        __shared__ int4 s_o[2][128];
        if constexpr (kFragEpi) setmaxnreg_dec<kWideProducerRegs>();
        const int pt = threadIdx.x - kConsumers;
        auto load_b = [&](int stage, int tap, int cb, int nt) {
            uint8_t *sb = smem + (size_t)stage * kStageBytes + (P.dcat ? 2 * kABytes : kABytes);
            const int wblk = (tap * P.cin_blocks + cb) * (P.split ? 2 : 1) * kBK;
            mbar_expect_tx(&full[stage], P.dcat ? 2 * kBBytes : kBBytes);
            tma_load_2d(sb, &P.tmB, &full[stage], wblk, nt * BN);
            if (P.dcat) tma_load_2d(sb + kBBytes, &P.tmB, &full[stage], wblk + kBK, nt * BN);
        };
        Ring r(stages);
        int tb = 0;
        for (int tile = blockIdx.x; tile < P.num_tiles; tile += gridDim.x) {
            int pi, wb, hb, ib, nt;
            decode_tile(P, tile, pi, wb, hb, ib, nt);
            const Problem &pr = P.prob[pi];
            const int taps = P.KH * P.KW;
            for (int tap = 0; tap < taps; ++tap) {
                if (pt < 128) {
                    const int iw = pt & (pr.BW - 1), ih = (pt >> pr.lbw) & (pr.BH - 1), ii = pt >> (pr.lbw + pr.lbh);
                    const int w = wb * pr.BW + iw, h = hb * pr.BH + ih, n = ib * pr.BI + ii;
                    const bool valid = (w < pr.Wo) && (h < pr.Ho) && (n < pr.N);
                    const size_t opix = ((size_t)(valid ? n : 0) * pr.Ho + (valid ? h : 0)) * pr.Wo + (valid ? w : 0);
                    const float *offp = pr.offset + opix * (2 * taps);
                    const float *mskp = pr.mask ? pr.mask + opix * taps : nullptr;
                    const int cpp = P.Cin * (SPLIT ? 2 : 1);
                    const int img0 = (valid ? n : 0) * pr.H * pr.W * cpp;
                    const int kh = tap / P.KW, kw = tap - kh * P.KW;
                    float4 wv = make_float4(0.f, 0.f, 0.f, 0.f);
                    int4 ov = make_int4(img0, img0, img0, img0);
                    if (valid) {
                        const float h_im = (float)(h * P.stride - P.pad + kh) + offp[2 * tap];
                        const float w_im = (float)(w * P.stride - P.pad + kw) + offp[2 * tap + 1];
                        if (h_im > -1.f && w_im > -1.f && h_im < (float)pr.H && w_im < (float)pr.W) {
                            const int h_low = (int)floorf(h_im), w_low = (int)floorf(w_im);
                            const int h_high = h_low + 1, w_high = w_low + 1;
                            const float lh = h_im - (float)h_low, lw = w_im - (float)w_low, hh = 1.f - lh, hw = 1.f - lw;
                            if (h_low >= 0 && w_low >= 0) { wv.x = hh * hw; ov.x = img0 + (h_low * pr.W + w_low) * cpp; }
                            if (h_low >= 0 && w_high <= pr.W - 1) { wv.y = hh * lw; ov.y = img0 + (h_low * pr.W + w_high) * cpp; }
                            if (h_high <= pr.H - 1 && w_low >= 0) { wv.z = lh * hw; ov.z = img0 + (h_high * pr.W + w_low) * cpp; }
                            if (h_high <= pr.H - 1 && w_high <= pr.W - 1) { wv.w = lh * lw; ov.w = img0 + (h_high * pr.W + w_high) * cpp; }
                            if (mskp) {
                                const float m = mskp[tap];
                                wv.x *= m; wv.y *= m; wv.z *= m; wv.w *= m;
                            }
                        }
                    }
                    s_w[tb][pt] = wv;
                    s_o[tb][pt] = ov;
                    if (P.split) {
                        const __half2 w01 = __floats2half2_rn(wv.x, wv.y), w23 = __floats2half2_rn(wv.z, wv.w);
                        s_wh[tb][pt] = make_uint2(*reinterpret_cast<const uint32_t *>(&w01), *reinterpret_cast<const uint32_t *>(&w23));
                    }
                }
                asm volatile("bar.sync 2, %0;" ::"n"(kDP) : "memory");
                for (int cb = 0; cb < P.cin_blocks; ++cb) {
                    if constexpr (!SPLIT) {
                        mbar_wait(&empty[r.stage], r.phase ^ 1);
                        if (pt == 0) load_b(r.stage, tap, cb, nt);
                        uint8_t *sa = smem + (size_t)r.stage * kStageBytes;
                        uint4 u[kDItems][4];
#pragma unroll
                        for (int it = 0; it < kDItems; ++it) {
                            const int item = pt + it * kDP, row = item >> 3, c16 = item & 7;
                            const int4 ov = s_o[tb][row];
                            const int co = cb * kBK + c16 * 8;
                            u[it][0] = *reinterpret_cast<const uint4 *>(pr.x + ov.x + co);
                            u[it][1] = *reinterpret_cast<const uint4 *>(pr.x + ov.y + co);
                            u[it][2] = *reinterpret_cast<const uint4 *>(pr.x + ov.z + co);
                            u[it][3] = *reinterpret_cast<const uint4 *>(pr.x + ov.w + co);
                        }
#pragma unroll
                        for (int it = 0; it < kDItems; ++it) {
                            const int item = pt + it * kDP, row = item >> 3, c16 = item & 7;
                            const float4 wv = s_w[tb][row];
                            const uint32_t *a1 = reinterpret_cast<const uint32_t *>(&u[it][0]);
                            const uint32_t *a2 = reinterpret_cast<const uint32_t *>(&u[it][1]);
                            const uint32_t *a3 = reinterpret_cast<const uint32_t *>(&u[it][2]);
                            const uint32_t *a4 = reinterpret_cast<const uint32_t *>(&u[it][3]);
                            uint32_t pk[4];
#pragma unroll
                            for (int k = 0; k < 4; ++k) {
                                const float2 f1 = __bfloat1622float2(*reinterpret_cast<const __nv_bfloat162 *>(&a1[k]));
                                const float2 f2 = __bfloat1622float2(*reinterpret_cast<const __nv_bfloat162 *>(&a2[k]));
                                const float2 f3 = __bfloat1622float2(*reinterpret_cast<const __nv_bfloat162 *>(&a3[k]));
                                const float2 f4 = __bfloat1622float2(*reinterpret_cast<const __nv_bfloat162 *>(&a4[k]));
                                const float vx = wv.x * f1.x + wv.y * f2.x + wv.z * f3.x + wv.w * f4.x;
                                const float vy = wv.x * f1.y + wv.y * f2.y + wv.z * f3.y + wv.w * f4.y;
                                __nv_bfloat162 b2 = __floats2bfloat162_rn(vx, vy);
                                pk[k] = *reinterpret_cast<uint32_t *>(&b2);
                            }
                            *reinterpret_cast<uint4 *>(sa + (size_t)row * 128 + ((c16 ^ (row & 7)) << 4)) = make_uint4(pk[0], pk[1], pk[2], pk[3]);
                        }
                        asm volatile("fence.proxy.async.shared::cta;" ::: "memory");
                        __syncwarp();
                        if ((pt & 31) == 0) mbar_arrive(&full[r.stage]);
                        r.next();
                    } else {
                        const __half *xh = reinterpret_cast<const __half *>(pr.x);
                        auto load_item = [&](int it, uint4 (&u)[4][2]) {
                            const int item = pt + it * kDP, row = item >> 3, c16 = item & 7;
                            const int4 ov = s_o[tb][row];
                            const int co = cb * kBK + c16 * 8;
                            const int oo[4] = {ov.x, ov.y, ov.z, ov.w};
#pragma unroll
                            for (int c = 0; c < 4; ++c) {
                                u[c][0] = *reinterpret_cast<const uint4 *>(xh + oo[c] + co);
                                u[c][1] = *reinterpret_cast<const uint4 *>(xh + oo[c] + P.Cin + co);
                            }
                        };
                        auto item_at = [&](int it) {
                            const int item = pt + it * kDP, row = item >> 3, c16 = item & 7;
                            return (uint32_t)(row * 128 + ((c16 ^ (row & 7)) << 4));
                        };
                        if constexpr (!kFragEpi) {
                            uint32_t phi[kDItems][4], plo[kDItems][4];
#pragma unroll
                            for (int i2 = 0; i2 < kDItems / kDRound; ++i2) {
                                uint4 u[kDRound][4][2];
#pragma unroll
                                for (int i1 = 0; i1 < kDRound; ++i1) load_item(i2 * kDRound + i1, u[i1]);
#pragma unroll
                                for (int i1 = 0; i1 < kDRound; ++i1) {
                                    const int it = i2 * kDRound + i1, row = (pt + it * kDP) >> 3;
                                    split_sample(u[i1], s_w[tb][row], s_wh[tb][row], phi[it], plo[it]);
                                }
                            }
                            mbar_wait(&empty[r.stage], r.phase ^ 1);
                            if (pt == 0) load_b(r.stage, tap, cb, nt);
                            uint8_t *sa = smem + (size_t)r.stage * kStageBytes;
#pragma unroll
                            for (int it = 0; it < kDItems; ++it) {
                                const uint32_t at = item_at(it);
                                *reinterpret_cast<uint4 *>(sa + at) = make_uint4(phi[it][0], phi[it][1], phi[it][2], phi[it][3]);
                                *reinterpret_cast<uint4 *>(sa + kABytes + at) = make_uint4(plo[it][0], plo[it][1], plo[it][2], plo[it][3]);
                            }
                        } else {
                            const uint32_t sa = smem_u32(smem + (size_t)r.stage * kStageBytes);
#pragma unroll
                            for (int i2 = 0; i2 < kDItems / kDRound; ++i2) {
                                uint4 u[kDRound][4][2];
#pragma unroll
                                for (int i1 = 0; i1 < kDRound; ++i1) load_item(i2 * kDRound + i1, u[i1]);
                                if (i2 == 0) {
                                    mbar_wait(&empty[r.stage], r.phase ^ 1);
                                    if (pt == 0) load_b(r.stage, tap, cb, nt);
                                }
#pragma unroll
                                for (int i1 = 0; i1 < kDRound; ++i1) {
                                    const int it = i2 * kDRound + i1, row = (pt + it * kDP) >> 3;
                                    uint32_t hi[4], lo[4];
                                    split_sample(u[i1], s_w[tb][row], s_wh[tb][row], hi, lo);
                                    const uint32_t at = sa + item_at(it);
                                    sts128(at, make_uint4(hi[0], hi[1], hi[2], hi[3]));
                                    sts128(at + kABytes, make_uint4(lo[0], lo[1], lo[2], lo[3]));
                                }
                            }
                        }
                        asm volatile("fence.proxy.async.shared::cta;" ::: "memory");
                        __syncwarp();
                        if ((pt & 31) == 0) mbar_arrive(&full[r.stage]);
                        r.next();
                    }
                }
                tb ^= 1;
            }
        }
    }
}

typedef CUresult (*EncodeTiledFn)(CUtensorMap *, CUtensorMapDataType, cuuint32_t, void *, const cuuint64_t *, const cuuint64_t *,
                                  const cuuint32_t *, const cuuint32_t *, CUtensorMapInterleave, CUtensorMapSwizzle,
                                  CUtensorMapL2promotion, CUtensorMapFloatOOBfill);

EncodeTiledFn encode_fn()
{
    static EncodeTiledFn fn = nullptr;
    static std::once_flag once;
    std::call_once(once, [] {
        void *p = nullptr;
        cudaDriverEntryPointQueryResult st;
        if (cudaGetDriverEntryPoint("cuTensorMapEncodeTiled", &p, cudaEnableDefault, &st) == cudaSuccess && st == cudaDriverEntryPointSuccess)
            fn = reinterpret_cast<EncodeTiledFn>(p);
    });
    return fn;
}

int pow2_floor(int v) { int p = 1; while (p * 2 <= v) p *= 2; return p; }

constexpr int kEvPool = 1024;
thread_local cudaEvent_t g_tc_ev[kEvPool][2];
thread_local int g_tc_ev_created = 0, g_tc_ev_used = 0;
thread_local double g_tc_flops = 0.0;
struct TcTrace { int nprob, N, H, W, Cin, Cout, K, stride, deform, BN, tiles, grid; double flops; };
thread_local TcTrace g_tc_trace[kEvPool];
thread_local orp_tc_plan g_tc_plan;
thread_local bool g_tc_plan_set = false;

constexpr int kSmemPerBlock = 227 * 1024;
constexpr int kStaticSmemPlain = 4096;
constexpr int kStaticSmemDeform = 14336;

struct ConvDesc {
    int nprob;
    const orp_tc_problem *probs;
    const void *w;
    int Cout, Cout_padded, KH, KW, Cin, stride, pad;
    const float *bias;
    int relu, out_f32, deform;
    int split;
    int wscale_log2;
    int stem;
    int ksplit;
};

struct ConvPlan {
    orp_tc_plan rep;
    Problem prob[kMaxProb];
    int num_m_tiles;
    int kbn;
    int extra_bytes;
};

int check_conv(const ConvDesc &d)
{
    if (d.split && (d.wscale_log2 < 0 || d.wscale_log2 > 15)) return fail(ORP_EINVAL, "conv2d_f16x3: weight scale exponent must be in 0..15");
    if (d.nprob < 1 || d.nprob > kMaxProb || !d.probs || !d.w) return fail(ORP_EINVAL, "conv2d_tc: bad arguments");
    if (d.Cin % 8) return fail(ORP_EINVAL, "conv2d_tc: Cin must be a multiple of 8 (16-byte channel rows)");
    if (d.deform && (d.Cin % kBK)) return fail(ORP_EINVAL, "conv2d_tc: deformable conv needs Cin % 64 == 0");
    if (d.Cout_padded % 32 || d.Cout_padded < d.Cout) return fail(ORP_EINVAL, "conv2d_tc: padded Cout must be a multiple of 32");
    if (d.stride < 1 || d.stride > 256) return fail(ORP_EINVAL, "conv2d_tc: stride must be in 1..256");
    if (d.deform)
        for (int i = 0; i < d.nprob; ++i)
            if ((long long)d.probs[i].N * d.probs[i].H * d.probs[i].W * d.Cin * (d.split ? 2 : 1) >= (1LL << 31))
                return fail(ORP_EINVAL, "conv2d_tc: deformable input has 2^31 or more 16-bit elements (32-bit sample offsets)");
    const orp_tc_problem &q0 = d.probs[0];
    if (d.ksplit > 1 && (d.nprob != 1 || d.deform || d.stem || !d.out_f32 || (d.KH * d.KW) % d.ksplit || q0.residual_bf16 ||
                         q0.residual_f32 || d.bias || d.relu))
        return fail(ORP_EINVAL, "conv2d_tc: split-K serves one plain problem with an fp32 partial-sum output and taps % ksplit == 0");
    return ORP_OK;
}

int plan_conv(const ConvDesc &d, int sms, ConvPlan &pl)
{
    int rc = check_conv(d);
    if (rc) return rc;
    memset(&pl, 0, sizeof(pl));
    const int nprob = d.nprob, ksplit = d.ksplit, T = d.split ? 2 : 1;
    const orp_tc_problem *probs = d.probs;

    int BN = 256;
    if (d.Cout_padded % 256) BN = (d.Cout_padded % 128 == 0) ? 128 : (d.Cout_padded % 64 == 0) ? 64 : 32;
    {
        long long mtiles = 0;
        for (int i = 0; i < nprob; ++i) {
            const int ho = (probs[i].H + 2 * d.pad - (d.KH - 1) - 1) / d.stride + 1, wo = (probs[i].W + 2 * d.pad - (d.KW - 1) - 1) / d.stride + 1;
            mtiles += ((long long)probs[i].N * ho * wo + 127) / 128;
        }
        while (BN > 64 && mtiles * (d.Cout_padded / BN) * ksplit < 120) BN /= 2;
    }
    if (d.deform && BN > 128) BN = 128;
    const int cin_blocks = (d.Cin + kBK - 1) / kBK;
    const int n_tiles_n = d.Cout_padded / BN;
    const int n_pair = (d.deform && d.split && !d.out_f32 && d.Cout % 8 == 0 && d.relu != 2 && BN == 128 && n_tiles_n % 2 == 0) ? 2 : 1;
    const int kbn = BN * n_pair;
    int mt = 0;
    for (int i = 0; i < nprob; ++i) {
        const orp_tc_problem &q = probs[i];
        Problem &pr = pl.prob[i];
        pr.N = q.N; pr.H = q.H; pr.W = q.W;
        pr.Ho = (q.H + 2 * d.pad - (d.KH - 1) - 1) / d.stride + 1;
        pr.Wo = (q.W + 2 * d.pad - (d.KW - 1) - 1) / d.stride + 1;
        if (pr.Ho <= 0 || pr.Wo <= 0 || !q.x || !q.out) return fail(ORP_EINVAL, "conv2d_tc: bad problem");
        pr.BW = pow2_floor(pr.Wo < 128 ? pr.Wo : 128);
        if (d.stride * pr.BW > 256) pr.BW = pow2_floor(256 / d.stride);
        pr.BH = pow2_floor(pr.Ho < 128 / pr.BW ? pr.Ho : 128 / pr.BW);
        pr.BI = 128 / (pr.BW * pr.BH);
        pr.lbw = 0; while ((1 << pr.lbw) < pr.BW) ++pr.lbw;
        pr.lbh = 0; while ((1 << pr.lbh) < pr.BH) ++pr.lbh;
        pr.tiles_w = ceil_div(pr.Wo, pr.BW); pr.tiles_h = ceil_div(pr.Ho, pr.BH); pr.tiles_i = ceil_div(pr.N, pr.BI);
        pr.tile_start = mt;
        pr.fd_tw.set((uint32_t)pr.tiles_w); pr.fd_th.set((uint32_t)pr.tiles_h);
        mt += pr.tiles_w * pr.tiles_h * pr.tiles_i;
        if (d.deform && !q.offset) return fail(ORP_EINVAL, "conv2d_tc: deformable conv needs offsets");
    }
    const int num_tiles = mt * n_tiles_n * ksplit;
    bool any_res = false;
    for (int i = 0; i < nprob; ++i) any_res = any_res || (probs[i].residual_bf16 != nullptr);
    const int tma_epi = (!d.out_f32 && ((d.Cout % 64 == 0) || (d.split && d.Cout % 8 == 0)) && BN >= 64) ? 1 : 0;
    if (d.split && !d.out_f32 && !tma_epi) return fail(ORP_EINVAL, "conv2d_f16x3: 16-bit outputs need Cout % 8 == 0 and weights padded to a multiple of 64 rows");
    if (d.split && d.out_f32 && any_res) return fail(ORP_EINVAL, "conv2d_f16x3: fp32 outputs take an fp32 residual only");
    const bool frag_epi = frag_epilogue(kbn, d.deform != 0);
    bool want_gn = false, gn_ok = tma_epi && d.Cout == 256 && !d.bias && !d.relu && !frag_epi;
    for (int i = 0; i < nprob; ++i) {
        want_gn = want_gn || (probs[i].gn_stats != nullptr);
        if (pl.prob[i].BW * pl.prob[i].BH < 32) gn_ok = false;
    }
    const int gn_fused = (want_gn && gn_ok) ? 1 : 0;
    const bool mem_bound = any_res || (d.KH * d.KW * (d.Cin / kBK) <= 8);
    int epi_bufs = mem_bound ? 2 : 1;
    const int epi_merge = (d.split && tma_epi && !frag_epi && (mem_bound || d.stem == 2)) ? 1 : 0;
    const int dcat = (d.split && d.deform) ? 1 : 0;
    const int ncat = (d.split && tma_epi && BN <= 128 && !d.deform && !any_res) ? 1 : 0;
    const int res_mma = (tma_epi && any_res) ? 1 : 0;
    if (res_mma) {
        if (d.deform) return fail(ORP_EINVAL, "conv2d_tc: residual is not supported on the deformable path");
        for (int i = 0; i < nprob; ++i)
            if (!probs[i].residual_bf16) return fail(ORP_EINVAL, "conv2d_tc: residual must be given for every problem or none");
    }
    const int slab_bytes = d.KH * d.KW * T * cin_blocks * BN * kBK * 2;
    int b_resident = (!d.deform && ksplit == 1 && slab_bytes <= 72 * 1024) ? 1 : 0;
    int grid = num_tiles / n_pair < sms ? num_tiles / n_pair : sms;
    if (b_resident && grid >= n_tiles_n) grid -= grid % n_tiles_n;
    else if (b_resident) b_resident = 0;
    int stage_b = 0, extra = 0, stages = 0;
    for (;;) {
        stage_b = stage_bytes(kbn, ncat || dcat, b_resident);
        const int hc = BN < 64 ? BN : 64;
        int staging = d.out_f32 ? 0 : 128 * (hc * 2 + 16);
        if (tma_epi) staging = epi_bufs * (epi_merge ? 32768 : 16384);
        extra = (res_mma ? 8192 : 0) + (b_resident ? slab_bytes : 0) + staging;
        stages = (kSmemPerBlock - (d.deform ? kStaticSmemDeform : kStaticSmemPlain) - dyn_smem_bytes(stage_b, 0, extra, frag_epi)) / stage_b;
        if (stages >= 3) break;
        if (epi_bufs == 2) { epi_bufs = 1; continue; }
        if (b_resident) { b_resident = 0; continue; }
        if (stages >= 2) break;
        return fail(ORP_EINVAL, "conv2d_tc: shared-memory budget cannot hold two main-loop stages");
    }
    if (stages > kStagesMax) stages = kStagesMax;
    if (d.deform && stages > 3) stages = 3;

    pl.num_m_tiles = mt;
    pl.kbn = kbn;
    pl.extra_bytes = extra;
    orp_tc_plan &r = pl.rep;
    r.BN = BN; r.stages = stages; r.grid = grid; r.num_tiles = num_tiles; r.n_tiles_n = n_tiles_n;
    r.ksplit = ksplit; r.nprob = nprob; r.Cout = d.Cout; r.Cout_padded = d.Cout_padded;
    r.split = d.split ? 1 : 0; r.deform = d.deform ? 1 : 0; r.out_f32 = d.out_f32 ? 1 : 0; r.stem = d.stem; r.relu = d.relu;
    r.bias = d.bias ? 1 : 0;
    for (int i = 0; i < nprob; ++i) {
        if (probs[i].residual_bf16) r.residual = 1;
        else if (probs[i].residual_f32) r.residual = 2;
        r.BW[i] = pl.prob[i].BW; r.BH[i] = pl.prob[i].BH; r.BI[i] = pl.prob[i].BI;
    }
    r.tma_epi = tma_epi; r.ncat = ncat; r.dcat = dcat; r.res_mma = res_mma; r.b_resident = b_resident;
    r.epi_merge = epi_merge; r.epi_bufs = epi_bufs; r.gn_fused = gn_fused; r.n_pair = n_pair;
    return ORP_OK;
}

int make_params(const ConvDesc &d, const ConvPlan &pl, TcParams &P)
{
    memset(&P, 0, sizeof(P));
    P.nprob = d.nprob; P.KH = d.KH; P.KW = d.KW; P.Cin = d.Cin; P.cin_blocks = (d.Cin + kBK - 1) / kBK;
    P.stride = d.stride; P.pad = d.pad;
    P.Cout = d.Cout; P.relu = d.relu; P.bias = d.bias; P.s2d_stem = (d.stem == 2) ? 1 : 0;
    P.split = d.split ? 1 : 0;
    P.oscale = d.split ? ldexpf(1.f, -d.wscale_log2) : 1.f;
    {
        void *ovf = nullptr;
        ORP_CUDA(cudaGetSymbolAddress(&ovf, g_f16_overflow));
        P.ovf = static_cast<unsigned int *>(ovf);
    }
    P.n_tiles_n = pl.rep.n_tiles_n / pl.rep.n_pair;
    P.fd_ntn.set((uint32_t)P.n_tiles_n);
    for (int i = 0; i < d.nprob; ++i) {
        const orp_tc_problem &q = d.probs[i];
        Problem &pr = P.prob[i];
        pr = pl.prob[i];
        pr.out = q.out; pr.res = static_cast<const __nv_bfloat16 *>(q.residual_bf16); pr.res32 = q.residual_f32;
        pr.x = static_cast<const __nv_bfloat16 *>(q.x); pr.offset = q.offset; pr.gn_stats = q.gn_stats; pr.mask = q.mask;
    }
    P.num_m_tiles = pl.num_m_tiles;
    P.num_tiles = pl.rep.num_tiles / pl.rep.n_pair;
    P.ksplit = d.ksplit;
    P.fd_ks.set((uint32_t)d.ksplit);
    P.ks_stride = (long long)P.prob[0].N * P.prob[0].Ho * P.prob[0].Wo * d.Cout;
    P.tma_epi = pl.rep.tma_epi; P.epi_bufs = pl.rep.epi_bufs; P.epi_merge = pl.rep.epi_merge; P.ncat = pl.rep.ncat;
    P.b_resident = pl.rep.b_resident; P.res_mma = pl.rep.res_mma; P.gn_fused = pl.rep.gn_fused; P.dcat = pl.rep.dcat;
    return ORP_OK;
}

int encode_maps(const ConvDesc &d, const ConvPlan &pl, TcParams &P)
{
    EncodeTiledFn enc = encode_fn();
    if (!enc) return fail(ORP_ECUDA, "conv2d_tc: cuTensorMapEncodeTiled unavailable");
    const CUtensorMapDataType dt16 = d.split ? CU_TENSOR_MAP_DATA_TYPE_FLOAT16 : CU_TENSOR_MAP_DATA_TYPE_BFLOAT16;
    const int T = d.split ? 2 : 1, Cin = d.Cin, Cout = d.Cout, stride = d.stride;
    if (!d.deform) {
        for (int i = 0; i < d.nprob; ++i) {
            const orp_tc_problem &q = d.probs[i];
            const Problem &pr = P.prob[i];
            cuuint64_t gdim[5] = {(cuuint64_t)Cin, (cuuint64_t)T, (cuuint64_t)q.W, (cuuint64_t)q.H, (cuuint64_t)q.N};
            cuuint64_t gstr[4] = {(cuuint64_t)Cin * 2, (cuuint64_t)Cin * 2 * T, (cuuint64_t)q.W * Cin * 2 * T,
                                  (cuuint64_t)q.H * q.W * Cin * 2 * T};
            if (d.stem == 2) {
                gstr[0] = (cuuint64_t)q.N * q.H * (q.W + 3) * 32;
                gstr[1] = 32;
                gstr[2] = (cuuint64_t)(q.W + 3) * 32;
                gstr[3] = (cuuint64_t)q.H * (q.W + 3) * 32;
            }
            cuuint32_t box[5] = {(cuuint32_t)kBK, 1u, (cuuint32_t)(pr.BW * stride), (cuuint32_t)(pr.BH * stride), (cuuint32_t)pr.BI};
            cuuint32_t estr[5] = {1, 1, (cuuint32_t)stride, (cuuint32_t)stride, 1};
            CUresult r = enc(&P.tmA[i], dt16, 5, const_cast<void *>(q.x), gdim, gstr, box, estr,
                             CU_TENSOR_MAP_INTERLEAVE_NONE, CU_TENSOR_MAP_SWIZZLE_128B, CU_TENSOR_MAP_L2_PROMOTION_L2_128B,
                             CU_TENSOR_MAP_FLOAT_OOB_FILL_NONE);
            if (r != CUDA_SUCCESS) return fail(ORP_ECUDA, "conv2d_tc: cuTensorMapEncodeTiled(A) failed");
        }
    }
    {
        const cuuint64_t K = (cuuint64_t)d.KH * d.KW * T * P.cin_blocks * kBK;
        cuuint64_t gdim[2] = {K, (cuuint64_t)d.Cout_padded};
        cuuint64_t gstr[1] = {K * 2};
        cuuint32_t box[2] = {(cuuint32_t)kBK, (cuuint32_t)pl.kbn};
        cuuint32_t estr[2] = {1, 1};
        CUresult r = enc(&P.tmB, dt16, 2, const_cast<void *>(d.w), gdim, gstr, box, estr,
                         CU_TENSOR_MAP_INTERLEAVE_NONE, CU_TENSOR_MAP_SWIZZLE_128B, CU_TENSOR_MAP_L2_PROMOTION_L2_256B,
                         CU_TENSOR_MAP_FLOAT_OOB_FILL_NONE);
        if (r != CUDA_SUCCESS) return fail(ORP_ECUDA, "conv2d_tc: cuTensorMapEncodeTiled(B) failed");
    }
    if (P.res_mma) {
        void *ident_ptr = nullptr;
        if (d.split) {
            ORP_CUDA(cudaGetSymbolAddress(&ident_ptr, g_ident16));
            ident_ptr = static_cast<char *>(ident_ptr) + (size_t)d.wscale_log2 * 8192;
        } else {
            ORP_CUDA(cudaGetSymbolAddress(&ident_ptr, g_ident));
        }
        cuuint64_t gdim[2] = {64, 64};
        cuuint64_t gstr[1] = {128};
        cuuint32_t box[2] = {64, 64};
        cuuint32_t estr[2] = {1, 1};
        CUresult r = enc(&P.tmI, dt16, 2, ident_ptr, gdim, gstr, box, estr, CU_TENSOR_MAP_INTERLEAVE_NONE,
                         CU_TENSOR_MAP_SWIZZLE_128B, CU_TENSOR_MAP_L2_PROMOTION_NONE, CU_TENSOR_MAP_FLOAT_OOB_FILL_NONE);
        if (r != CUDA_SUCCESS) return fail(ORP_ECUDA, "conv2d_tc: cuTensorMapEncodeTiled(identity) failed");
    }
    if (P.tma_epi) {
        for (int i = 0; i < d.nprob; ++i) {
            const Problem &pr = P.prob[i];
            cuuint64_t gdim[5] = {(cuuint64_t)Cout, (cuuint64_t)T, (cuuint64_t)pr.Wo, (cuuint64_t)pr.Ho, (cuuint64_t)pr.N};
            cuuint64_t gstr[4] = {(cuuint64_t)Cout * 2, (cuuint64_t)Cout * 2 * T, (cuuint64_t)pr.Wo * Cout * 2 * T,
                                  (cuuint64_t)pr.Ho * pr.Wo * Cout * 2 * T};
            cuuint32_t box[5] = {64u, 1u, (cuuint32_t)pr.BW, (cuuint32_t)pr.BH, (cuuint32_t)pr.BI};
            cuuint32_t estr[5] = {1, 1, 1, 1, 1};
            CUresult r = enc(&P.tmOut[i], dt16, 5, pr.out, gdim, gstr, box, estr,
                             CU_TENSOR_MAP_INTERLEAVE_NONE, CU_TENSOR_MAP_SWIZZLE_128B, CU_TENSOR_MAP_L2_PROMOTION_NONE,
                             CU_TENSOR_MAP_FLOAT_OOB_FILL_NONE);
            if (r != CUDA_SUCCESS) return fail(ORP_ECUDA, "conv2d_tc: cuTensorMapEncodeTiled(out) failed");
            if (pr.res) {
                r = enc(&P.tmRes[i], dt16, 5, const_cast<__nv_bfloat16 *>(pr.res), gdim, gstr, box, estr,
                        CU_TENSOR_MAP_INTERLEAVE_NONE, CU_TENSOR_MAP_SWIZZLE_128B, CU_TENSOR_MAP_L2_PROMOTION_L2_128B,
                        CU_TENSOR_MAP_FLOAT_OOB_FILL_NONE);
                if (r != CUDA_SUCCESS) return fail(ORP_ECUDA, "conv2d_tc: cuTensorMapEncodeTiled(residual) failed");
            }
        }
    }
    return ORP_OK;
}

template <int BN, bool OUT_F32, bool DEFORM, bool SPLIT, int WALK>
int launch_tc(const TcParams &P, int stages, int grid, cudaStream_t st, int extra_bytes)
{
    constexpr bool kCat = WALK == kWalkNcat || WALK == kWalkDcat;
    const int smem = dyn_smem_bytes(stage_bytes(BN, kCat, P.b_resident), stages, extra_bytes, frag_epilogue(BN, DEFORM));
    auto kern = conv_tc_kernel<BN, OUT_F32, DEFORM, SPLIT, WALK>;
    static int smem_max = -1;
    if (smem_max < 0) {
        cudaFuncAttributes fa;
        ORP_CUDA(cudaFuncGetAttributes(&fa, kern));
        ORP_CUDA(cudaFuncSetAttribute(kern, cudaFuncAttributeMaxDynamicSharedMemorySize, kSmemPerBlock - (int)fa.sharedSizeBytes));
        smem_max = kSmemPerBlock - (int)fa.sharedSizeBytes;
    }
    if (smem > smem_max) {
        char need[32];
        snprintf(need, sizeof(need), "%d", smem);
        return fail(ORP_EINVAL, "conv2d_tc: the plan's %s bytes of dynamic shared memory do not fit beside the static shared memory of %s",
                    need, __PRETTY_FUNCTION__);
    }
    int slot = -1;
    if (g_timing && g_tc_ev_used < kEvPool) {
        slot = g_tc_ev_used++;
        if (slot >= g_tc_ev_created) {
            ORP_CUDA(cudaEventCreate(&g_tc_ev[slot][0]));
            ORP_CUDA(cudaEventCreate(&g_tc_ev[slot][1]));
            g_tc_ev_created = slot + 1;
        }
        ORP_CUDA(cudaEventRecord(g_tc_ev[slot][0], st));
        double fl = 0;
        for (int i = 0; i < P.nprob; ++i)
            fl += 2.0 * P.prob[i].N * P.prob[i].Ho * P.prob[i].Wo * (double)P.Cout *
                  (P.s2d_stem ? 147.0 : (double)P.KH * P.KW * P.Cin);
        g_tc_flops += fl;
        g_tc_trace[slot] = TcTrace{P.nprob, P.prob[0].N, P.prob[0].H, P.prob[0].W, P.Cin, P.Cout, P.KH, P.stride, DEFORM ? 1 : 0,
                                   BN, P.num_tiles, grid, fl};
    }
    {
        cudaLaunchConfig_t cfg;
        memset(&cfg, 0, sizeof(cfg));
        cfg.gridDim = dim3((unsigned)grid);
        cfg.blockDim = dim3(DEFORM ? (unsigned)(kConsumers + kDP) : (unsigned)(kConsumers + 128));
        cfg.dynamicSmemBytes = smem;
        cfg.stream = st;
        cudaLaunchAttribute at[1];
        at[0].id = cudaLaunchAttributeProgrammaticStreamSerialization;
        at[0].val.programmaticStreamSerializationAllowed = 1;
        cfg.attrs = at;
        cfg.numAttrs = 1;
        ORP_CUDA(cudaLaunchKernelEx(&cfg, kern, P, stages));
    }
    ORP_LAUNCHED();
    if (slot >= 0) ORP_CUDA(cudaEventRecord(g_tc_ev[slot][1], st));
    return ORP_OK;
}

template <int BN, bool OUT_F32, bool DEFORM>
int launch_plan(const TcParams &P, int stages, int grid, cudaStream_t st, int extra_bytes)
{
    if constexpr (DEFORM) {
        if (P.dcat != P.split || P.ncat || P.res_mma) return fail(ORP_EINVAL, "conv2d_tc: deformable plan outside dcat == split");
        if constexpr (frag_epilogue(BN, true)) {
            if (!P.split || OUT_F32 || !P.tma_epi || P.epi_merge || P.gn_fused || P.relu == 2)
                return fail(ORP_EINVAL, "conv2d_tc: deformable N-tile pair outside f16x3 with an unmerged TMA epilogue and no GELU");
            return launch_tc<BN, false, true, true, kWalkDcat>(P, stages, grid, st, extra_bytes);
        } else {
            return P.split ? launch_tc<BN, OUT_F32, true, true, kWalkDcat>(P, stages, grid, st, extra_bytes)
                           : launch_tc<BN, OUT_F32, true, false, kWalkK>(P, stages, grid, st, extra_bytes);
        }
    } else {
        if (P.ncat && P.res_mma) return fail(ORP_EINVAL, "conv2d_tc: ncat plan with a residual");
        if (P.ncat) {
            if constexpr (!OUT_F32 && BN >= 64 && BN <= 128) {
                if (P.split) return launch_tc<BN, false, false, true, kWalkNcat>(P, stages, grid, st, extra_bytes);
            }
            return fail(ORP_EINVAL, "conv2d_tc: ncat plan outside f16x3 TMA-epilogue layers with BN 64..128");
        }
        if (P.res_mma) {
            if constexpr (!OUT_F32 && BN >= 64)
                return P.split ? launch_tc<BN, false, false, true, kWalkKRes>(P, stages, grid, st, extra_bytes)
                               : launch_tc<BN, false, false, false, kWalkKRes>(P, stages, grid, st, extra_bytes);
            return fail(ORP_EINVAL, "conv2d_tc: residual K blocks outside TMA-epilogue layers with BN >= 64");
        }
        return P.split ? launch_tc<BN, OUT_F32, false, true, kWalkK>(P, stages, grid, st, extra_bytes)
                       : launch_tc<BN, OUT_F32, false, false, kWalkK>(P, stages, grid, st, extra_bytes);
    }
}

template <bool OUT_F32, bool DEFORM>
int launch_bn(const TcParams &P, const ConvPlan &pl, cudaStream_t st)
{
    const int s = pl.rep.stages, g = pl.rep.grid, e = pl.extra_bytes;
    switch (pl.kbn) {
    case 256:
        if constexpr (!DEFORM || !OUT_F32) return launch_plan<256, OUT_F32, DEFORM>(P, s, g, st, e);
        break;
    case 128: return launch_plan<128, OUT_F32, DEFORM>(P, s, g, st, e);
    case 64: return launch_plan<64, OUT_F32, DEFORM>(P, s, g, st, e);
    case 32: return launch_plan<32, OUT_F32, DEFORM>(P, s, g, st, e);
    }
    return fail(ORP_EINVAL, "conv2d_tc: unsupported tile width");
}

int device_sms(int &sms)
{
    static thread_local int dev_known = -1, sms_known = 0;
    int dev = 0;
    ORP_CUDA(cudaGetDevice(&dev));
    if (dev != dev_known) {
        ORP_CUDA(cudaDeviceGetAttribute(&sms_known, cudaDevAttrMultiProcessorCount, dev));
        dev_known = dev;
    }
    sms = sms_known;
    return ORP_OK;
}

int conv2d_tc(const ConvDesc &d, void *stream)
{
    int rc = check_conv(d);
    if (rc) return rc;
    rc = ensure_device();
    if (rc) return rc;
    int sms = 0;
    rc = device_sms(sms);
    if (rc) return rc;
    ConvPlan pl;
    rc = plan_conv(d, sms, pl);
    if (rc) return rc;
    TcParams P;
    rc = make_params(d, pl, P);
    if (rc) return rc;
    rc = encode_maps(d, pl, P);
    if (rc) return rc;
    g_tc_plan = pl.rep;
    g_tc_plan_set = true;
    cudaStream_t st = static_cast<cudaStream_t>(stream);
    rc = d.out_f32 ? (d.deform ? launch_bn<true, true>(P, pl, st) : launch_bn<true, false>(P, pl, st))
                   : (d.deform ? launch_bn<false, true>(P, pl, st) : launch_bn<false, false>(P, pl, st));
    if (rc) return rc;
    bool want_gn = false;
    for (int i = 0; i < d.nprob; ++i) want_gn = want_gn || (d.probs[i].gn_stats != nullptr);
    if (want_gn && !P.gn_fused) {
        if (d.out_f32 || d.Cout != 256) return fail(ORP_EINVAL, "conv2d_tc: gn_stats needs a 16-bit output with 256 channels");
        for (int i = 0; i < d.nprob; ++i)
            if (d.probs[i].gn_stats) {
                int r2 = d.split ? orp_gn_stats_f16x3(P.prob[i].out, P.prob[i].N, P.prob[i].Ho * P.prob[i].Wo, 256, 32, d.probs[i].gn_stats, stream)
                                 : orp_gn_stats_bf16(P.prob[i].out, P.prob[i].N, P.prob[i].Ho * P.prob[i].Wo, 256, 32, d.probs[i].gn_stats, stream);
                if (r2) return r2;
            }
    }
    return ORP_OK;
}

int stem_desc(const void *x_s2d, int N, int H, int W, const void *w, const float *bias, int relu, void *out, int split,
              int wscale_log2, orp_tc_problem &q, ConvDesc &d)
{
    if (!x_s2d || !w || !out || N < 1 || H < 2 || W < 2 || (H & 1) || (W & 1))
        return fail(ORP_EINVAL, "stem_conv_s2d_%s: needs even H, W", split ? "f16x3" : "bf16");
    if (split && (wscale_log2 < 0 || wscale_log2 > 15)) return fail(ORP_EINVAL, "stem_conv_s2d_f16x3: weight scale exponent must be in 0..15");
    memset(&q, 0, sizeof(q));
    q.x = x_s2d;
    q.N = N; q.H = H / 2 + 3; q.W = W / 2; q.out = out;
    d = ConvDesc{1, &q, w, 64, 64, 4, 1, 64, 1, 0, bias, relu, 0, 0, split, split ? wscale_log2 : 0, 2, 1};
    return ORP_OK;
}

int splitk_desc(const orp_tc_problem *prob, const void *w, int Cout, int Cout_padded, int KH, int KW, int Cin, int stride, int pad,
                int f16x3, int wscale_log2, int ksplit, void *workspace, orp_tc_problem &q, ConvDesc &d, int &Ho, int &Wo)
{
    if (!prob || !w || !workspace || ksplit < 2 || (Cout % 8)) return fail(ORP_EINVAL, "conv2d_tc_splitk: bad arguments");
    if (f16x3 && (wscale_log2 < 0 || wscale_log2 > 15)) return fail(ORP_EINVAL, "conv2d_tc_splitk: weight scale exponent must be in 0..15");
    Ho = (prob->H + 2 * pad - (KH - 1) - 1) / stride + 1;
    Wo = (prob->W + 2 * pad - (KW - 1) - 1) / stride + 1;
    if (Ho <= 0 || Wo <= 0) return fail(ORP_EINVAL, "conv2d_tc_splitk: bad problem");
    q = *prob;
    q.out = workspace;
    q.gn_stats = nullptr;
    d = ConvDesc{1, &q, w, Cout, Cout_padded, KH, KW, Cin, stride, pad, nullptr, 0, 1, 0, f16x3 ? 1 : 0, wscale_log2, 0, ksplit};
    return ORP_OK;
}

__global__ void __launch_bounds__(256)
splitk_finish_kernel(const float *__restrict__ ws, int ksplit, size_t pixels, int C, const float *__restrict__ bias, int relu, int split,
                     void *__restrict__ out, unsigned int *ovf)
{
    const int c8 = C / 8;
    const size_t total = pixels * c8;
    for (size_t i = blockIdx.x * (size_t)blockDim.x + threadIdx.x; i < total; i += (size_t)gridDim.x * blockDim.x) {
        const size_t pix = i / c8;
        const int c = (int)(i - pix * c8) * 8;
        float v[8] = {0.f, 0.f, 0.f, 0.f, 0.f, 0.f, 0.f, 0.f};
        for (int k = 0; k < ksplit; ++k) {
            const float *p = ws + (size_t)k * pixels * C + pix * C + c;
            const float4 a = *reinterpret_cast<const float4 *>(p), b = *reinterpret_cast<const float4 *>(p + 4);
            v[0] += a.x; v[1] += a.y; v[2] += a.z; v[3] += a.w; v[4] += b.x; v[5] += b.y; v[6] += b.z; v[7] += b.w;
        }
        float amax = 0.f;
#pragma unroll
        for (int j = 0; j < 8; ++j) {
            if (bias) v[j] += bias[c + j];
            if (relu) v[j] = fmaxf(v[j], 0.f);
            amax = fmaxf(amax, fabsf(v[j]));
        }
        uint32_t hi[4], lo[4];
        if (split) {
#pragma unroll
            for (int k = 0; k < 4; ++k) {
                const __half2 h2 = __floats2half2_rn(v[2 * k], v[2 * k + 1]);
                const float2 hf = __half22float2(h2);
                const __half2 l2 = __floats2half2_rn(v[2 * k] - hf.x, v[2 * k + 1] - hf.y);
                hi[k] = *reinterpret_cast<const uint32_t *>(&h2);
                lo[k] = *reinterpret_cast<const uint32_t *>(&l2);
            }
            __half *o = static_cast<__half *>(out) + pix * 2 * C + c;
            *reinterpret_cast<uint4 *>(o) = make_uint4(hi[0], hi[1], hi[2], hi[3]);
            *reinterpret_cast<uint4 *>(o + C) = make_uint4(lo[0], lo[1], lo[2], lo[3]);
            if (amax > 65504.f) atomicAdd(ovf, 1u);
        } else {
#pragma unroll
            for (int k = 0; k < 4; ++k) {
                __nv_bfloat162 b2 = __floats2bfloat162_rn(v[2 * k], v[2 * k + 1]);
                hi[k] = *reinterpret_cast<uint32_t *>(&b2);
            }
            *reinterpret_cast<uint4 *>(static_cast<__nv_bfloat16 *>(out) + pix * C + c) = make_uint4(hi[0], hi[1], hi[2], hi[3]);
        }
    }
}
}
}

using namespace orp;

extern "C" int orp_tc_timing_collect(float *total_ms, int *launches, double *flops)
{
    if (!total_ms || !launches || !flops) return fail(ORP_EINVAL, "orp_tc_timing_collect: null");
    float sum = 0.f;
    for (int i = 0; i < g_tc_ev_used; ++i) {
        float ms = 0.f;
        ORP_CUDA(cudaEventSynchronize(g_tc_ev[i][1]));
        ORP_CUDA(cudaEventElapsedTime(&ms, g_tc_ev[i][0], g_tc_ev[i][1]));
        sum += ms;
        if (getenv("ORP_TC_TRACE")) {
            const TcTrace &t = g_tc_trace[i];
            fprintf(stderr, "tc[%3d] np=%d N=%d %4dx%-4d Cin=%4d Cout=%4d k=%d s=%d dcn=%d BN=%3d tiles=%5d grid=%3d  %8.1f us  %7.1f TFLOP/s\n",
                    i, t.nprob, t.N, t.H, t.W, t.Cin, t.Cout, t.K, t.stride, t.deform, t.BN, t.tiles, t.grid, ms * 1e3,
                    t.flops / (ms * 1e-3) / 1e12);
        }
    }
    *total_ms = sum; *launches = g_tc_ev_used; *flops = g_tc_flops;
    g_tc_ev_used = 0; g_tc_flops = 0.0;
    return ORP_OK;
}

extern "C" int orp_tc_last_plan(orp_tc_plan *out)
{
    if (!out) return fail(ORP_EINVAL, "orp_tc_last_plan: null");
    if (!g_tc_plan_set) return fail(ORP_EINVAL, "orp_tc_last_plan: no tensor-core convolution launched on this thread");
    *out = g_tc_plan;
    return ORP_OK;
}

extern "C" int orp_tc_plan_conv(int nprob, const orp_tc_problem *probs, const void *w, int Cout, int Cout_padded, int KH, int KW,
                                int Cin, int stride, int pad, const float *bias, int wscale_log2, int relu, int out_f32, int deform,
                                int split, int stem, int ksplit, int sms, orp_tc_plan *out)
{
    if (!out || sms < 1 || (stem != 0 && stem != 2)) return fail(ORP_EINVAL, "orp_tc_plan_conv: bad arguments");
    split = split ? 1 : 0;
    orp_tc_problem q;
    ConvDesc d;
    int rc = ORP_OK;
    if (stem == 2 || ksplit > 1) {
        if (nprob != 1 || !probs || deform || out_f32 || (stem == 2 && ksplit > 1))
            return fail(ORP_EINVAL, "orp_tc_plan_conv: the stem and split-K plan one problem with a 16-bit output");
        int Ho, Wo;
        rc = stem == 2 ? stem_desc(probs->x, probs->N, probs->H, probs->W, w, bias, relu, probs->out, split, wscale_log2, q, d)
                       : splitk_desc(probs, w, Cout, Cout_padded, KH, KW, Cin, stride, pad, split, wscale_log2, ksplit, probs->out, q,
                                     d, Ho, Wo);
    } else {
        d = ConvDesc{nprob, probs, w, Cout, Cout_padded, KH, KW, Cin, stride, pad, bias, relu, out_f32, deform, split, wscale_log2, 0, 1};
    }
    if (rc) return rc;
    ConvPlan pl;
    rc = plan_conv(d, sms, pl);
    if (rc) return rc;
    *out = pl.rep;
    return ORP_OK;
}

extern "C" int orp_conv2d_bf16(int nprob, const orp_tc_problem *probs, const void *w, int Cout, int Cout_padded, int KH,
                               int KW, int Cin, int stride, int pad, const float *bias, int relu, int out_f32,
                               int deform, void *stream)
{
    return conv2d_tc(ConvDesc{nprob, probs, w, Cout, Cout_padded, KH, KW, Cin, stride, pad, bias, relu, out_f32, deform, 0, 0, 0, 1},
                     stream);
}

extern "C" int orp_conv2d_f16x3(int nprob, const orp_tc_problem *probs, const void *w_split, int Cout, int Cout_padded, int KH,
                                int KW, int Cin, int stride, int pad, const float *bias, int wscale_log2, int relu,
                                int out_f32, int deform, void *stream)
{
    return conv2d_tc(ConvDesc{nprob, probs, w_split, Cout, Cout_padded, KH, KW, Cin, stride, pad, bias, relu, out_f32, deform, 1,
                              wscale_log2, 0, 1},
                     stream);
}

extern "C" int orp_stem_conv_s2d_f16x3(const void *x_s2d, int N, int H, int W, const void *w_split, const float *bias,
                                       int wscale_log2, int relu, void *out, void *stream)
{
    orp_tc_problem q;
    ConvDesc d;
    const int rc = stem_desc(x_s2d, N, H, W, w_split, bias, relu, out, 1, wscale_log2, q, d);
    return rc ? rc : conv2d_tc(d, stream);
}

extern "C" int orp_stem_conv_s2d_bf16(const void *x_s2d, int N, int H, int W, const void *w256, const float *bias, int relu,
                                      void *out, void *stream)
{
    orp_tc_problem q;
    ConvDesc d;
    const int rc = stem_desc(x_s2d, N, H, W, w256, bias, relu, out, 0, 0, q, d);
    return rc ? rc : conv2d_tc(d, stream);
}

__global__ void overflow_take_kernel(unsigned int *dst, int reset)
{
    *dst = reset ? atomicExch(&g_f16_overflow, 0u) : atomicAdd(&g_f16_overflow, 0u);
}

extern "C" int orp_f16x3_overflow_count(unsigned int *count, int reset, void *stream)
{
    if (!count) return fail(ORP_EINVAL, "f16x3_overflow_count: null");
    static thread_local unsigned int *host = nullptr;
    static thread_local unsigned int *dev = nullptr;
    if (!host) {
        ORP_CUDA(cudaHostAlloc(reinterpret_cast<void **>(&host), sizeof(unsigned int), cudaHostAllocMapped));
        ORP_CUDA(cudaHostGetDevicePointer(reinterpret_cast<void **>(&dev), host, 0));
    }
    cudaStream_t st = static_cast<cudaStream_t>(stream);
    overflow_take_kernel<<<1, 1, 0, st>>>(dev, reset ? 1 : 0);
    ORP_LAUNCHED();
    ORP_CUDA(cudaStreamSynchronize(st));
    *count = *host;
    return ORP_OK;
}

extern "C" int orp_conv2d_tc_splitk(const orp_tc_problem *prob, const void *w, int Cout, int Cout_padded, int KH, int KW, int Cin,
                                    int stride, int pad, const float *bias, int f16x3, int wscale_log2, int relu, int ksplit,
                                    float *workspace, void *stream)
{
    orp_tc_problem q;
    ConvDesc d;
    int Ho = 0, Wo = 0;
    int rc = splitk_desc(prob, w, Cout, Cout_padded, KH, KW, Cin, stride, pad, f16x3, wscale_log2, ksplit, workspace, q, d, Ho, Wo);
    if (rc) return rc;
    rc = conv2d_tc(d, stream);
    if (rc) return rc;
    cudaStream_t st = static_cast<cudaStream_t>(stream);
    const size_t pixels = (size_t)prob->N * Ho * Wo;
    void *ovf = nullptr;
    ORP_CUDA(cudaGetSymbolAddress(&ovf, g_f16_overflow));
    splitk_finish_kernel<<<grid_for(pixels * (Cout / 8), 256), 256, 0, st>>>(workspace, ksplit, pixels, Cout, bias, relu, f16x3 ? 1 : 0, prob->out,
                                                                static_cast<unsigned int *>(ovf));
    ORP_LAUNCHED();
    if (prob->gn_stats) {
        if (Cout != 256) return fail(ORP_EINVAL, "conv2d_tc_splitk: gn_stats needs 256 output channels");
        return f16x3 ? orp_gn_stats_f16x3(prob->out, prob->N, Ho * Wo, 256, 32, prob->gn_stats, stream)
                     : orp_gn_stats_bf16(prob->out, prob->N, Ho * Wo, 256, 32, prob->gn_stats, stream);
    }
    return ORP_OK;
}
```

Before: 320.6.

## Write TMA epilogue directly from accumulator fragments and reuse accumulator region as output slots

Extends the fragment-based epilogue, which skips staging accumulators through shared memory, from the deformable N-tile pair case to all TMA-epilogue tiles with BN up to 128. The shared accumulator region is then reused as extra TMA output staging slots, and spare shared memory adds more slots, up to four in flight. This removes a staging round-trip and barriers and deepens the store pipeline. In exchange it adds register pressure and complexity, including GroupNorm stats exchange and ncat summation now handled in fragments.

```diff
diff --git a/include/orp_b200.h b/include/orp_b200.h
--- a/include/orp_b200.h
+++ b/include/orp_b200.h
@@ -86,6 +86,8 @@
     int tma_epi, ncat, dcat, res_mma, b_resident, epi_merge, epi_bufs, gn_fused;
     int BW[5], BH[5], BI[5];
     int n_pair;
+    int frag_epi;
+    int epi_slots;
 } orp_tc_plan;
 int orp_tc_last_plan(orp_tc_plan *out);
 
diff --git a/orientedreppoints_b200/_lib.py b/orientedreppoints_b200/_lib.py
--- a/orientedreppoints_b200/_lib.py
+++ b/orientedreppoints_b200/_lib.py
@@ -43,7 +43,7 @@
     _fields_ = [(k, _i) for k in ("BN", "stages", "grid", "num_tiles", "n_tiles_n", "ksplit", "nprob", "Cout", "Cout_padded",
                                   "split", "deform", "out_f32", "stem", "relu", "bias", "residual", "tma_epi", "ncat", "dcat",
                                   "res_mma", "b_resident", "epi_merge", "epi_bufs", "gn_fused")] + \
-              [(k, _i * 5) for k in ("BW", "BH", "BI")] + [("n_pair", _i)]
+              [(k, _i * 5) for k in ("BW", "BH", "BI")] + [("n_pair", _i), ("frag_epi", _i), ("epi_slots", _i)]
 
     def as_dict(self):
         d = {k: getattr(self, k) for k, _ in self._fields_}
diff --git a/orientedreppoints_b200/csrc/dense_tc.cu b/orientedreppoints_b200/csrc/dense_tc.cu
--- a/orientedreppoints_b200/csrc/dense_tc.cu
+++ b/orientedreppoints_b200/csrc/dense_tc.cu
@@ -55,6 +55,8 @@
     CUtensorMap tmI;
     Problem prob[kMaxProb];
     int tma_epi, epi_bufs;
+    int epi_slots;
+    int epi_out;
     int epi_merge;
     int ncat;
     int ksplit;
@@ -280,14 +282,25 @@
 {
     return cat ? (b_resident ? 2 * kABytes : 2 * kABytes + 2 * BN * kBK * 2) : (b_resident ? kABytes : kABytes + BN * kBK * 2);
 }
-__host__ __device__ constexpr bool frag_epilogue(int BN, bool deform) { return deform && BN == 256; }
-constexpr int dyn_smem_bytes(int stage_b, int stages, int extra, bool frag_epi)
-{
-    return 1024 + (frag_epi ? 0 : kAccBytes) + stages * stage_b + extra;
-}
+__host__ __device__ constexpr bool pair_variant(int BN, bool deform) { return deform && BN == 256; }
+constexpr int dyn_smem_bytes(int stage_b, int stages, int extra, bool pair)
+{
+    return 1024 + (pair ? 0 : kAccBytes) + stages * stage_b + extra;
+}
+__host__ __device__ constexpr bool frag_epilogue(int BN, bool deform) { return BN <= 128 || pair_variant(BN, deform); }
+constexpr int kGnRowBytes = 128 * 8 * 8;
+constexpr int kGnPitch = 20;
+constexpr int kGnWarpBytes = 16 * kGnPitch * 4;
+constexpr int kGnBytes = kGnRowBytes + 8 * kGnWarpBytes;
+__host__ __device__ constexpr int region_slots(bool pair, bool merge, bool gn)
+{
+    return pair ? 0 : (kAccBytes - (gn ? kGnBytes : 0)) / (merge ? 32768 : 16384);
+}
+static_assert(region_slots(false, false, false) == 2 && region_slots(false, false, true) == 1 && region_slots(false, true, false) == 1,
+              "accumulator region: two 16 KiB slots, one beside the GroupNorm exchange, or one merged 32 KiB slot");
 
 template <int BN, int R>
-__device__ __forceinline__ void stage_acc(const float (&acc)[R], int pass, bool ncat, float *s_acc, int row0, int col0)
+__device__ __forceinline__ void stage_acc(const float (&acc)[R], int pass, float *s_acc, int row0, int col0)
 {
     constexpr int kGroups = (BN < 64 ? BN : 64) / 8;
 #pragma unroll
@@ -296,17 +309,18 @@
 #pragma unroll
         for (int i = 0; i < kGroups; ++i) {
             const int g = p * 8 + i;
-            float2 a = make_float2(acc[4 * g], acc[4 * g + 1]), b = make_float2(acc[4 * g + 2], acc[4 * g + 3]);
-            if constexpr (R >= BN) {
-                if (ncat) {
-                    a.x += acc[BN / 2 + 4 * g]; a.y += acc[BN / 2 + 4 * g + 1];
-                    b.x += acc[BN / 2 + 4 * g + 2]; b.y += acc[BN / 2 + 4 * g + 3];
-                }
-            }
-            *reinterpret_cast<float2 *>(s_acc + row0 * kAccPitch + i * 8 + col0) = a;
-            *reinterpret_cast<float2 *>(s_acc + (row0 + 8) * kAccPitch + i * 8 + col0) = b;
-        }
-    }
+            *reinterpret_cast<float2 *>(s_acc + row0 * kAccPitch + i * 8 + col0) = make_float2(acc[4 * g], acc[4 * g + 1]);
+            *reinterpret_cast<float2 *>(s_acc + (row0 + 8) * kAccPitch + i * 8 + col0) = make_float2(acc[4 * g + 2], acc[4 * g + 3]);
+        }
+    }
+}
+
+__device__ __forceinline__ void bulk_wait_read(int pending)
+{
+    if (pending >= 3) asm volatile("cp.async.bulk.wait_group.read 3;" ::: "memory");
+    else if (pending == 2) asm volatile("cp.async.bulk.wait_group.read 2;" ::: "memory");
+    else if (pending == 1) asm volatile("cp.async.bulk.wait_group.read 1;" ::: "memory");
+    else asm volatile("cp.async.bulk.wait_group.read 0;" ::: "memory");
 }
 
 constexpr int kWalkK = 0;
@@ -350,8 +364,9 @@
     constexpr bool kCat = WALK == kWalkNcat || WALK == kWalkDcat;
     constexpr int kKMode = (SPLIT && !kCat) ? 1 : 0;
     static_assert(kConsumers + 128 == 384 && 2 * 128 * kConsumerRegs + 128 * kProducerRegs <= 65536, "register split");
-    constexpr bool kFragEpi = frag_epilogue(BN, DEFORM);
-    static_assert(!kFragEpi || (SPLIT && !OUT_F32), "fragment epilogue: deformable f16x3 with a TMA epilogue");
+    constexpr bool kPair = pair_variant(BN, DEFORM);
+    constexpr bool kFragEpi = !OUT_F32 && frag_epilogue(BN, DEFORM);
+    static_assert(!kPair || (SPLIT && !OUT_F32), "N-tile pairs: deformable f16x3 with a TMA epilogue");
     static_assert(kConsumers == 256 && kDP == 256 && 2 * 128 * kWideConsumerRegs + 2 * 128 * kWideProducerRegs <= 65536,
                   "register split (wide deformable)");
     constexpr int kEpiThreads = kConsumers;
@@ -360,7 +375,7 @@
     extern __shared__ __align__(1024) uint8_t smem_raw[];
     uint8_t *smem = reinterpret_cast<uint8_t *>((reinterpret_cast<uintptr_t>(smem_raw) + 1023) & ~uintptr_t(1023));
     float *s_acc = reinterpret_cast<float *>(smem);
-    if constexpr (!kFragEpi) smem += kAccBytes;
+    if constexpr (!kPair) smem += kAccBytes;
     constexpr int kBBytes = BN * kBK * 2;
     const int kStageBytes = stage_bytes(BN, kCat, P.b_resident);
     const int kblocks_all = P.KH * P.KW * P.cin_blocks * kWTerms;
@@ -406,7 +421,7 @@
 
     if (warp < kConsumers / 32) {
         if constexpr (!DEFORM) setmaxnreg_inc<kConsumerRegs>();
-        if constexpr (kFragEpi) setmaxnreg_inc<kWideConsumerRegs>();
+        if constexpr (kPair) setmaxnreg_inc<kWideConsumerRegs>();
         const int cw = warp >> 2;
         const uint32_t a_off = (uint32_t)cw * 8192u;
         const bool leader = (threadIdx.x & 127) == 0;
@@ -436,7 +451,7 @@
                 held = next;
             };
             for (int kb = 0; kb < kblocks; ++kb, it.next()) {
-                if constexpr (kFragEpi) {
+                if constexpr (kPair) {
                     wgmma_wait<0>();
                     release(-1);
                 }
@@ -524,74 +539,11 @@
             };
             size_t pix;
             const bool valid = row_pixel(rrow, pix);
-            if constexpr (kFragEpi) {
-                const uint32_t obuf_u = smem_u32(stage_out);
-                const bool io = (et == 0);
-                if (nt != bias_nt) {
-                    bar_sync(bar_a, nthr);
-                    for (int c = et; c < BN; c += nthr) s_bias[c] = (P.bias && nt * BN + c < P.Cout) ? P.bias[nt * BN + c] : 0.f;
-                    bias_nt = nt;
-                }
-                size_t pix_r[2];
-                const bool valid_r[2] = {row_pixel(frow, pix_r[0]), row_pixel(frow + 8, pix_r[1])};
-                float amax[2][2] = {{0.f, 0.f}, {0.f, 0.f}};
-#pragma unroll
-                for (int pass = 0; pass < 2 * (BN / 64); ++pass) {
-                    const int half = pass >> 1, oterm = pass & 1;
-                    if (io) {
-                        if (P.epi_bufs == 2) asm volatile("cp.async.bulk.wait_group.read 1;" ::: "memory");
-                        else asm volatile("cp.async.bulk.wait_group.read 0;" ::: "memory");
-                    }
-                    bar_sync(bar_a, nthr);
-                    const uint32_t obase = obuf_u + (uint32_t)ob * 16384u;
-#pragma unroll
-                    for (int i = 0; i < 8; ++i) {
-                        const int g = half * 8 + i;
-                        const float2 bv = *reinterpret_cast<const float2 *>(&s_bias[g * 8 + fcol]);
-#pragma unroll
-                        for (int hr = 0; hr < 2; ++hr) {
-                            const int row = frow + 8 * hr;
-                            float f0 = acc[4 * g + 2 * hr], f1 = acc[4 * g + 2 * hr + 1];
-                            f0 *= P.oscale; f1 *= P.oscale;
-                            f0 += bv.x; f1 += bv.y;
-                            if (P.relu) { f0 = fmaxf(f0, 0.f); f1 = fmaxf(f1, 0.f); }
-                            if (oterm == 0) amax[hr][i >> 2] = fmaxf(fmaxf(amax[hr][i >> 2], fabsf(f0)), fabsf(f1));
-                            const __half2 h2 = __floats2half2_rn(f0, f1);
-                            uint32_t v = *reinterpret_cast<const uint32_t *>(&h2);
-                            if (oterm) {
-                                const float2 hf = __half22float2(h2);
-                                const __half2 l2 = __floats2half2_rn(f0 - hf.x, f1 - hf.y);
-                                v = *reinterpret_cast<const uint32_t *>(&l2);
-                            }
-                            const uint32_t at = obase + (uint32_t)row * 128u + ((uint32_t)(i ^ (row & 7)) << 4) + (uint32_t)fcol * 2u;
-                            asm volatile("st.shared.b32 [%0], %1;" ::"r"(at), "r"(v) : "memory");
-                        }
-                    }
-                    asm volatile("fence.proxy.async.shared::cta;" ::: "memory");
-                    bar_sync(bar_b, nthr);
-                    if (io) {
-                        asm volatile(
-                            "cp.async.bulk.tensor.5d.global.shared::cta.bulk_group [%0, {%2, %3, %4, %5, %6}], [%1];"
-                            ::"l"(&P.tmOut[pi]), "r"(obase), "r"(nt * BN + half * 64), "r"(oterm),
-                              "r"(wb * pr.BW), "r"(hb * pr.BH), "r"(ib * pr.BI) : "memory");
-                        asm volatile("cp.async.bulk.commit_group;" ::: "memory");
-                    }
-                    if (++ob == P.epi_bufs) ob = 0;
-                }
-#pragma unroll
-                for (int hr = 0; hr < 2; ++hr)
-#pragma unroll
-                    for (int hc = 0; hc < 2; ++hc) {
-                        float m = amax[hr][hc];
-                        m = fmaxf(m, __shfl_xor_sync(0xffffffffu, m, 1));
-                        m = fmaxf(m, __shfl_xor_sync(0xffffffffu, m, 2));
-                        if ((lane & 3) == 0 && valid_r[hr] && m > 65504.f) atomicAdd(P.ovf, 1u);
-                    }
-            } else if (OUT_F32) {
+            if constexpr (OUT_F32) {
 #pragma unroll 1
                 for (int pass = 0; pass < BN / HC; ++pass) {
                 bar_sync(bar_a, nthr);
-                stage_acc<BN>(acc, pass, false, s_acc, frow, fcol);
+                stage_acc<BN>(acc, pass, s_acc, frow, fcol);
                 bar_sync(bar_a, nthr);
 #pragma unroll 1
                 for (int ch = wg; ch < HC / 32; ch += kWG) {
@@ -620,129 +572,266 @@
                     }
                 }
                 }
-            } else if (P.tma_epi) {
-                const uint32_t slot = P.epi_merge ? 32768u : 16384u;
-                const uint32_t obuf_u = smem_u32(stage_out);
-                const uint32_t bias_u = smem_u32(s_bias);
-                const bool io = (et == 0);
-                constexpr int kPasses = BN / 64;
-                const int oterms = (P.split && !P.epi_merge) ? 2 : 1;
-                if (nt != bias_nt) {
-                    bar_sync(bar_a, nthr);
-                    for (int c = et; c < BN; c += nthr) s_bias[c] = (P.bias && nt * BN + c < P.Cout) ? P.bias[nt * BN + c] : 0.f;
-                    bias_nt = nt;
-                }
-                float amax = 0.f;
-#pragma unroll 1
-                for (int pass = 0; pass < kPasses * oterms; ++pass) {
-                    const int half = oterms == 2 ? (pass >> 1) : pass, oterm = oterms == 2 ? (pass & 1) : 0;
-                    if (io) {
-                        if (P.epi_bufs == 2) asm volatile("cp.async.bulk.wait_group.read 1;" ::: "memory");
-                        else asm volatile("cp.async.bulk.wait_group.read 0;" ::: "memory");
+            } else if (kPair || P.tma_epi) {
+                if constexpr (kFragEpi) {
+                    constexpr bool kFull = !kPair;
+                    const bool merge = kFull && P.epi_merge;
+                    const uint32_t slot = merge ? 32768u : 16384u;
+                    const uint32_t obuf_u = smem_u32(stage_out);
+                    const uint32_t gn_u = s_acc_u + (uint32_t)(P.epi_slots - P.epi_out) * slot;
+                    const uint32_t gsc_u = gn_u + kGnRowBytes + (uint32_t)warp * kGnWarpBytes;
+                    const bool io = (et == 0);
+                    const int oterms = (SPLIT && !merge) ? 2 : 1;
+                    if (nt != bias_nt) {
+                        bar_sync(bar_a, nthr);
+                        for (int c = et; c < BN; c += nthr) s_bias[c] = (P.bias && nt * BN + c < P.Cout) ? P.bias[nt * BN + c] : 0.f;
+                        bias_nt = nt;
                     }
-                    bar_sync(bar_a, nthr);
-                    if (oterm == 0) {
-                        stage_acc<BN>(acc, half, P.ncat != 0, s_acc, frow, fcol);
-                        bar_sync(bar_a, nthr);
-                    }
-                    float gn_s = 0.f, gn_q = 0.f;
-                    const uint32_t orow = obuf_u + (uint32_t)ob * slot + (uint32_t)rrow * 128u;
-#pragma unroll 1
-                    for (int ch = ch0; ch < 2; ch += chs) {
-                        const uint32_t arow = s_acc_u + (uint32_t)(rrow * kAccPitch + ch * 32) * 4u;
-#pragma unroll
-                        for (int j4 = 0; j4 < 4; ++j4) {
-                            const int c16 = ch * 4 + j4;
-                            const uint32_t sw = (uint32_t)(c16 ^ (rrow & 7)) << 4;
-                            const uint4 a0 = lds128(arow + (uint32_t)j4 * 32u), a1 = lds128(arow + (uint32_t)j4 * 32u + 16u);
-                            const float f0[8] = {__uint_as_float(a0.x), __uint_as_float(a0.y), __uint_as_float(a0.z), __uint_as_float(a0.w),
-                                                 __uint_as_float(a1.x), __uint_as_float(a1.y), __uint_as_float(a1.z), __uint_as_float(a1.w)};
-                            float f[8];
-#pragma unroll
-                            for (int j = 0; j < 8; ++j) f[j] = f0[j];
-                            const uint32_t bb = bias_u + (uint32_t)(half * 64 + ch * 32 + j4 * 8) * 4u;
-                            const uint4 b0 = lds128(bb), b1 = lds128(bb + 16u);
-                            if (P.split) {
-#pragma unroll
-                                for (int j = 0; j < 8; ++j) f[j] *= P.oscale;
-                            }
-                            f[0] += __uint_as_float(b0.x); f[1] += __uint_as_float(b0.y);
-                            f[2] += __uint_as_float(b0.z); f[3] += __uint_as_float(b0.w);
-                            f[4] += __uint_as_float(b1.x); f[5] += __uint_as_float(b1.y);
-                            f[6] += __uint_as_float(b1.z); f[7] += __uint_as_float(b1.w);
-                            if (P.relu == 2) {
-#pragma unroll
-                                for (int j = 0; j < 8; ++j) f[j] = act_fn(f[j], 2);
-                            }
-                            uint32_t pk[4];
-                            if (P.split) {
-#pragma unroll
-                                for (int j = 0; j < 8; ++j) {
-                                    if (P.relu == 1) f[j] = fmaxf(f[j], 0.f);
-                                    if (oterm == 0) amax = fmaxf(amax, fabsf(f[j]));
-                                }
-                                uint32_t pl[4];
-#pragma unroll
-                                for (int k = 0; k < 4; ++k) {
-                                    const __half2 h2 = __floats2half2_rn(f[2 * k], f[2 * k + 1]);
-                                    pk[k] = *reinterpret_cast<const uint32_t *>(&h2);
-                                    if (P.epi_merge || oterm) {
-                                        const float2 hf = __half22float2(h2);
-                                        const __half2 l2 = __floats2half2_rn(f[2 * k] - hf.x, f[2 * k + 1] - hf.y);
-                                        pl[k] = *reinterpret_cast<const uint32_t *>(&l2);
+                    size_t pix_r[2];
+                    const bool valid_r[2] = {row_pixel(frow, pix_r[0]), row_pixel(frow + 8, pix_r[1])};
+                    const int gn_row = cw * 64 + q * 16 + (lane & 15);
+                    size_t gn_pix;
+                    const bool gn_valid = row_pixel(gn_row, gn_pix);
+                    float amax[2][2] = {{0.f, 0.f}, {0.f, 0.f}};
+#pragma unroll
+                    for (int half = 0; half < BN / 64; ++half) {
+#pragma unroll
+                        for (int oterm = 0; oterm < (SPLIT ? 2 : 1); ++oterm) {
+                            if (oterm >= oterms) break;
+                            if (io) bulk_wait_read(P.epi_slots - 1);
+                            bar_sync(bar_a, nthr);
+                            const uint32_t obase = (kPair || ob < P.epi_out) ? obuf_u + (uint32_t)ob * slot : s_acc_u + (uint32_t)(ob - P.epi_out) * slot;
+                            const bool gn = kFull && P.gn_fused && oterm == 0;
+#pragma unroll
+                            for (int i2 = 0; i2 < 4; ++i2) {
+#pragma unroll
+                                for (int i1 = 0; i1 < 2; ++i1) {
+                                    const int i = 2 * i2 + i1;
+                                    const int g = half * 8 + i;
+                                    const float2 bv = *reinterpret_cast<const float2 *>(&s_bias[g * 8 + fcol]);
+#pragma unroll
+                                    for (int hr = 0; hr < 2; ++hr) {
+                                        const int row = frow + 8 * hr;
+                                        float f0 = acc[4 * g + 2 * hr], f1 = acc[4 * g + 2 * hr + 1];
+                                        if constexpr (WALK == kWalkNcat) {
+                                            f0 += acc[BN / 2 + 4 * g + 2 * hr];
+                                            f1 += acc[BN / 2 + 4 * g + 2 * hr + 1];
+                                        }
+                                        if constexpr (SPLIT) { f0 *= P.oscale; f1 *= P.oscale; }
+                                        f0 += bv.x; f1 += bv.y;
+                                        if (kFull && P.relu == 2) { f0 = act_fn(f0, 2); f1 = act_fn(f1, 2); }
+                                        const uint32_t at = obase + (uint32_t)row * 128u + ((uint32_t)(i ^ (row & 7)) << 4) + (uint32_t)fcol * 2u;
+                                        uint32_t v;
+                                        if constexpr (SPLIT) {
+                                            if (P.relu == 1) { f0 = fmaxf(f0, 0.f); f1 = fmaxf(f1, 0.f); }
+                                            if (oterm == 0) amax[hr][i >> 2] = fmaxf(fmaxf(amax[hr][i >> 2], fabsf(f0)), fabsf(f1));
+                                            const __half2 h2 = __floats2half2_rn(f0, f1);
+                                            v = *reinterpret_cast<const uint32_t *>(&h2);
+                                            if (merge || oterm) {
+                                                const float2 hf = __half22float2(h2);
+                                                const __half2 l2 = __floats2half2_rn(f0 - hf.x, f1 - hf.y);
+                                                const uint32_t vl = *reinterpret_cast<const uint32_t *>(&l2);
+                                                if (merge) asm volatile("st.shared.b32 [%0], %1;" ::"r"(at + 16384u), "r"(vl) : "memory");
+                                                else v = vl;
+                                            }
+                                        } else {
+                                            __nv_bfloat162 b2 = __floats2bfloat162_rn(f0, f1);
+                                            if (P.relu == 1) b2 = __hmax2(b2, __floats2bfloat162_rn(0.f, 0.f));
+                                            v = *reinterpret_cast<const uint32_t *>(&b2);
+                                        }
+                                        asm volatile("st.shared.b32 [%0], %1;" ::"r"(at), "r"(v) : "memory");
+                                        if (gn) {
+                                            const uint32_t sc = gsc_u + (uint32_t)(((lane >> 2) + 8 * hr) * kGnPitch + i1 * 8 + fcol) * 4u;
+                                            asm volatile("st.shared.v2.f32 [%0], {%1, %2};" ::"r"(sc), "f"(f0), "f"(f1) : "memory");
+                                        }
                                     }
                                 }
-                                if (P.epi_merge) sts128(orow + 16384u + sw, make_uint4(pl[0], pl[1], pl[2], pl[3]));
-                                else if (oterm) { pk[0] = pl[0]; pk[1] = pl[1]; pk[2] = pl[2]; pk[3] = pl[3]; }
-                            } else {
+                                if (gn) {
+                                    __syncwarp();
+                                    const uint4 a0 = lds128(gsc_u + (uint32_t)((lane & 15) * kGnPitch + (lane >> 4) * 8) * 4u);
+                                    const uint4 a1 = lds128(gsc_u + (uint32_t)((lane & 15) * kGnPitch + (lane >> 4) * 8 + 4) * 4u);
+                                    const float fv[8] = {__uint_as_float(a0.x), __uint_as_float(a0.y), __uint_as_float(a0.z), __uint_as_float(a0.w),
+                                                         __uint_as_float(a1.x), __uint_as_float(a1.y), __uint_as_float(a1.z), __uint_as_float(a1.w)};
+                                    float gs = 0.f, gq = 0.f;
+                                    if (gn_valid) {
+#pragma unroll
+                                        for (int j = 0; j < 8; ++j) { gs += fv[j]; gq = fmaf(fv[j], fv[j], gq); }
+                                    }
+                                    const uint32_t gp = gn_u + (uint32_t)((2 * i2 + (lane >> 4)) * 128 + gn_row) * 8u;
+                                    asm volatile("st.shared.v2.f32 [%0], {%1, %2};" ::"r"(gp), "f"(gs), "f"(gq) : "memory");
+                                    __syncwarp();
+                                }
+                            }
+                            asm volatile("fence.proxy.async.shared::cta;" ::: "memory");
+                            bar_sync(bar_b, nthr);
+                            if (io) {
+                                asm volatile(
+                                    "cp.async.bulk.tensor.5d.global.shared::cta.bulk_group [%0, {%2, %3, %4, %5, %6}], [%1];"
+                                    ::"l"(&P.tmOut[pi]), "r"(obase), "r"(nt * BN + half * 64), "r"(oterm),
+                                      "r"(wb * pr.BW), "r"(hb * pr.BH), "r"(ib * pr.BI) : "memory");
+                                if (merge)
+                                    asm volatile(
+                                        "cp.async.bulk.tensor.5d.global.shared::cta.bulk_group [%0, {%2, %3, %4, %5, %6}], [%1];"
+                                        ::"l"(&P.tmOut[pi]), "r"(obase + 16384u), "r"(nt * BN + half * 64), "r"(1),
+                                          "r"(wb * pr.BW), "r"(hb * pr.BH), "r"(ib * pr.BI) : "memory");
+                                asm volatile("cp.async.bulk.commit_group;" ::: "memory");
+                            }
+                            if (gn) {
+                                float gn_s = 0.f, gn_q = 0.f;
 #pragma unroll
                                 for (int k = 0; k < 4; ++k) {
-                                    __nv_bfloat162 b2 = __floats2bfloat162_rn(f[2 * k], f[2 * k + 1]);
-                                    if (P.relu == 1) b2 = __hmax2(b2, __floats2bfloat162_rn(0.f, 0.f));
-                                    pk[k] = *reinterpret_cast<uint32_t *>(&b2);
+                                    float gs, gq;
+                                    asm volatile("ld.shared.v2.f32 {%0, %1}, [%2];" : "=f"(gs), "=f"(gq)
+                                                 : "r"(gn_u + (uint32_t)((wg * 4 + k) * 128 + q * 32 + lane) * 8u) : "memory");
+#pragma unroll
+                                    for (int o = 16; o > 0; o >>= 1) {
+                                        gs += __shfl_xor_sync(0xffffffffu, gs, o);
+                                        gq += __shfl_xor_sync(0xffffffffu, gq, o);
+                                    }
+                                    if (lane == k) { gn_s = gs; gn_q = gq; }
                                 }
-                            }
-                            sts128(orow + sw, make_uint4(pk[0], pk[1], pk[2], pk[3]));
-                            if (P.gn_fused && oterm == 0) {
-                                float gs = 0.f, gq = 0.f;
-                                if (valid) {
-#pragma unroll
-                                    for (int j = 0; j < 8; ++j) { gs += f[j]; gq = fmaf(f[j], f[j], gq); }
+                                const int n_img = ib * pr.BI + ((q * 32) >> (pr.lbw + pr.lbh));
+                                if (lane < 4 && n_img < pr.N) {
+                                    double *st = pr.gn_stats + ((size_t)n_img * 32 + (size_t)(nt * BN + half * 64) / 8 + wg * 4 + lane) * 2;
+                                    atomicAdd(st, (double)gn_s);
+                                    atomicAdd(st + 1, (double)gn_q);
                                 }
-#pragma unroll
-                                for (int o = 16; o > 0; o >>= 1) {
-                                    gs += __shfl_xor_sync(0xffffffffu, gs, o);
-                                    gq += __shfl_xor_sync(0xffffffffu, gq, o);
-                                }
-                                if (lane == c16) { gn_s = gs; gn_q = gq; }
-                            }
+                            }
+                            if (++ob == P.epi_slots) ob = 0;
                         }
                     }
-                    if (P.gn_fused && oterm == 0 && lane < 8 && (chs == 1 || (lane >> 2) == wg)) {
-                        const int n_img = ib * pr.BI + ((q * 32) >> (pr.lbw + pr.lbh));
-                        if (n_img < pr.N) {
-                            double *st = pr.gn_stats + ((size_t)n_img * 32 + (size_t)(nt * BN + half * 64) / 8 + lane) * 2;
-                            atomicAdd(st, (double)gn_s);
-                            atomicAdd(st + 1, (double)gn_q);
+                    if constexpr (SPLIT) {
+#pragma unroll
+                        for (int hr = 0; hr < 2; ++hr)
+#pragma unroll
+                            for (int hc = 0; hc < 2; ++hc) {
+                                float m = amax[hr][hc];
+                                m = fmaxf(m, __shfl_xor_sync(0xffffffffu, m, 1));
+                                m = fmaxf(m, __shfl_xor_sync(0xffffffffu, m, 2));
+                                if ((lane & 3) == 0 && valid_r[hr] && m > 65504.f) atomicAdd(P.ovf, 1u);
+                            }
+                    }
+                } else {
+                    const uint32_t slot = P.epi_merge ? 32768u : 16384u;
+                    const uint32_t obuf_u = smem_u32(stage_out);
+                    const uint32_t bias_u = smem_u32(s_bias);
+                    const bool io = (et == 0);
+                    constexpr int kPasses = BN / 64;
+                    const int oterms = (P.split && !P.epi_merge) ? 2 : 1;
+                    if (nt != bias_nt) {
+                        bar_sync(bar_a, nthr);
+                        for (int c = et; c < BN; c += nthr) s_bias[c] = (P.bias && nt * BN + c < P.Cout) ? P.bias[nt * BN + c] : 0.f;
+                        bias_nt = nt;
+                    }
+                    float amax = 0.f;
+#pragma unroll 1
+                    for (int pass = 0; pass < kPasses * oterms; ++pass) {
+                        const int half = oterms == 2 ? (pass >> 1) : pass, oterm = oterms == 2 ? (pass & 1) : 0;
+                        if (io) bulk_wait_read(P.epi_slots - 1);
+                        bar_sync(bar_a, nthr);
+                        if (oterm == 0) {
+                            stage_acc<BN>(acc, half, s_acc, frow, fcol);
+                            bar_sync(bar_a, nthr);
                         }
-                    }
-                    asm volatile("fence.proxy.async.shared::cta;" ::: "memory");
-                    bar_sync(bar_b, nthr);
-                    if (io) {
-                        asm volatile(
-                            "cp.async.bulk.tensor.5d.global.shared::cta.bulk_group [%0, {%2, %3, %4, %5, %6}], [%1];"
-                            ::"l"(&P.tmOut[pi]), "r"(obuf_u + (uint32_t)ob * slot), "r"(nt * BN + half * 64), "r"(oterm),
-                              "r"(wb * pr.BW), "r"(hb * pr.BH), "r"(ib * pr.BI) : "memory");
-                        if (P.epi_merge)
+                        float gn_s = 0.f, gn_q = 0.f;
+                        const uint32_t orow = obuf_u + (uint32_t)ob * slot + (uint32_t)rrow * 128u;
+#pragma unroll 1
+                        for (int ch = ch0; ch < 2; ch += chs) {
+                            const uint32_t arow = s_acc_u + (uint32_t)(rrow * kAccPitch + ch * 32) * 4u;
+#pragma unroll
+                            for (int j4 = 0; j4 < 4; ++j4) {
+                                const int c16 = ch * 4 + j4;
+                                const uint32_t sw = (uint32_t)(c16 ^ (rrow & 7)) << 4;
+                                const uint4 a0 = lds128(arow + (uint32_t)j4 * 32u), a1 = lds128(arow + (uint32_t)j4 * 32u + 16u);
+                                const float f0[8] = {__uint_as_float(a0.x), __uint_as_float(a0.y), __uint_as_float(a0.z), __uint_as_float(a0.w),
+                                                     __uint_as_float(a1.x), __uint_as_float(a1.y), __uint_as_float(a1.z), __uint_as_float(a1.w)};
+                                float f[8];
+#pragma unroll
+                                for (int j = 0; j < 8; ++j) f[j] = f0[j];
+                                const uint32_t bb = bias_u + (uint32_t)(half * 64 + ch * 32 + j4 * 8) * 4u;
+                                const uint4 b0 = lds128(bb), b1 = lds128(bb + 16u);
+                                if (P.split) {
+#pragma unroll
+                                    for (int j = 0; j < 8; ++j) f[j] *= P.oscale;
+                                }
+                                f[0] += __uint_as_float(b0.x); f[1] += __uint_as_float(b0.y);
+                                f[2] += __uint_as_float(b0.z); f[3] += __uint_as_float(b0.w);
+                                f[4] += __uint_as_float(b1.x); f[5] += __uint_as_float(b1.y);
+                                f[6] += __uint_as_float(b1.z); f[7] += __uint_as_float(b1.w);
+                                if (P.relu == 2) {
+#pragma unroll
+                                    for (int j = 0; j < 8; ++j) f[j] = act_fn(f[j], 2);
+                                }
+                                uint32_t pk[4];
+                                if (P.split) {
+#pragma unroll
+                                    for (int j = 0; j < 8; ++j) {
+                                        if (P.relu == 1) f[j] = fmaxf(f[j], 0.f);
+                                        if (oterm == 0) amax = fmaxf(amax, fabsf(f[j]));
+                                    }
+                                    uint32_t pl[4];
+#pragma unroll
+                                    for (int k = 0; k < 4; ++k) {
+                                        const __half2 h2 = __floats2half2_rn(f[2 * k], f[2 * k + 1]);
+                                        pk[k] = *reinterpret_cast<const uint32_t *>(&h2);
+                                        if (P.epi_merge || oterm) {
+                                            const float2 hf = __half22float2(h2);
+                                            const __half2 l2 = __floats2half2_rn(f[2 * k] - hf.x, f[2 * k + 1] - hf.y);
+                                            pl[k] = *reinterpret_cast<const uint32_t *>(&l2);
+                                        }
+                                    }
+                                    if (P.epi_merge) sts128(orow + 16384u + sw, make_uint4(pl[0], pl[1], pl[2], pl[3]));
+                                    else if (oterm) { pk[0] = pl[0]; pk[1] = pl[1]; pk[2] = pl[2]; pk[3] = pl[3]; }
+                                } else {
+#pragma unroll
+                                    for (int k = 0; k < 4; ++k) {
+                                        __nv_bfloat162 b2 = __floats2bfloat162_rn(f[2 * k], f[2 * k + 1]);
+                                        if (P.relu == 1) b2 = __hmax2(b2, __floats2bfloat162_rn(0.f, 0.f));
+                                        pk[k] = *reinterpret_cast<uint32_t *>(&b2);
+                                    }
+                                }
+                                sts128(orow + sw, make_uint4(pk[0], pk[1], pk[2], pk[3]));
+                                if (P.gn_fused && oterm == 0) {
+                                    float gs = 0.f, gq = 0.f;
+                                    if (valid) {
+#pragma unroll
+                                        for (int j = 0; j < 8; ++j) { gs += f[j]; gq = fmaf(f[j], f[j], gq); }
+                                    }
+#pragma unroll
+                                    for (int o = 16; o > 0; o >>= 1) {
+                                        gs += __shfl_xor_sync(0xffffffffu, gs, o);
+                                        gq += __shfl_xor_sync(0xffffffffu, gq, o);
+                                    }
+                                    if (lane == c16) { gn_s = gs; gn_q = gq; }
+                                }
+                            }
+                        }
+                        if (P.gn_fused && oterm == 0 && lane < 8 && (chs == 1 || (lane >> 2) == wg)) {
+                            const int n_img = ib * pr.BI + ((q * 32) >> (pr.lbw + pr.lbh));
+                            if (n_img < pr.N) {
+                                double *st = pr.gn_stats + ((size_t)n_img * 32 + (size_t)(nt * BN + half * 64) / 8 + lane) * 2;
+                                atomicAdd(st, (double)gn_s);
+                                atomicAdd(st + 1, (double)gn_q);
+                            }
+                        }
+                        asm volatile("fence.proxy.async.shared::cta;" ::: "memory");
+                        bar_sync(bar_b, nthr);
+                        if (io) {
                             asm volatile(
                                 "cp.async.bulk.tensor.5d.global.shared::cta.bulk_group [%0, {%2, %3, %4, %5, %6}], [%1];"
-                                ::"l"(&P.tmOut[pi]), "r"(obuf_u + (uint32_t)ob * slot + 16384u), "r"(nt * BN + half * 64), "r"(1),
+                                ::"l"(&P.tmOut[pi]), "r"(obuf_u + (uint32_t)ob * slot), "r"(nt * BN + half * 64), "r"(oterm),
                                   "r"(wb * pr.BW), "r"(hb * pr.BH), "r"(ib * pr.BI) : "memory");
-                        asm volatile("cp.async.bulk.commit_group;" ::: "memory");
+                            if (P.epi_merge)
+                                asm volatile(
+                                    "cp.async.bulk.tensor.5d.global.shared::cta.bulk_group [%0, {%2, %3, %4, %5, %6}], [%1];"
+                                    ::"l"(&P.tmOut[pi]), "r"(obuf_u + (uint32_t)ob * slot + 16384u), "r"(nt * BN + half * 64), "r"(1),
+                                      "r"(wb * pr.BW), "r"(hb * pr.BH), "r"(ib * pr.BI) : "memory");
+                            asm volatile("cp.async.bulk.commit_group;" ::: "memory");
+                        }
+                        if (++ob == P.epi_slots) ob = 0;
                     }
-                    if (++ob == P.epi_bufs) ob = 0;
+                    if (P.split && valid && amax > 65504.f) atomicAdd(P.ovf, 1u);
                 }
-                if (P.split && valid && amax > 65504.f) atomicAdd(P.ovf, 1u);
             } else {
                 const bool vec_ok = (P.Cout & 7) == 0;
                 named_bar<1, kEpiThreads>();
@@ -766,7 +855,7 @@
                         asm volatile("cp.async.commit_group;" ::: "memory");
                     }
                     if (pr.res && vec_ok) asm volatile("cp.async.wait_group 0;" ::: "memory");
-                    stage_acc<BN>(acc, half, false, s_acc, frow, fcol);
+                    stage_acc<BN>(acc, half, s_acc, frow, fcol);
                     named_bar<1, kEpiThreads>();
 #pragma unroll 1
                     for (int ch = wg; ch < HC / 32; ch += kWG) {
@@ -888,7 +977,7 @@
         __shared__ float4 s_w[2][128];
         __shared__ uint2 s_wh[2][128];
         __shared__ int4 s_o[2][128];
-        if constexpr (kFragEpi) setmaxnreg_dec<kWideProducerRegs>();
+        if constexpr (kPair) setmaxnreg_dec<kWideProducerRegs>();
         const int pt = threadIdx.x - kConsumers;
         auto load_b = [&](int stage, int tap, int cb, int nt) {
             uint8_t *sb = smem + (size_t)stage * kStageBytes + (P.dcat ? 2 * kABytes : kABytes);
@@ -1001,7 +1090,7 @@
                             const int item = pt + it * kDP, row = item >> 3, c16 = item & 7;
                             return (uint32_t)(row * 128 + ((c16 ^ (row & 7)) << 4));
                         };
-                        if constexpr (!kFragEpi) {
+                        if constexpr (!kPair) {
                             uint32_t phi[kDItems][4], plo[kDItems][4];
 #pragma unroll
                             for (int i2 = 0; i2 < kDItems / kDRound; ++i2) {
@@ -1108,6 +1197,7 @@
     int num_m_tiles;
     int kbn;
     int extra_bytes;
+    int epi_out;
 };
 
 int check_conv(const ConvDesc &d)
@@ -1178,8 +1268,8 @@
     const int tma_epi = (!d.out_f32 && ((d.Cout % 64 == 0) || (d.split && d.Cout % 8 == 0)) && BN >= 64) ? 1 : 0;
     if (d.split && !d.out_f32 && !tma_epi) return fail(ORP_EINVAL, "conv2d_f16x3: 16-bit outputs need Cout % 8 == 0 and weights padded to a multiple of 64 rows");
     if (d.split && d.out_f32 && any_res) return fail(ORP_EINVAL, "conv2d_f16x3: fp32 outputs take an fp32 residual only");
-    const bool frag_epi = frag_epilogue(kbn, d.deform != 0);
-    bool want_gn = false, gn_ok = tma_epi && d.Cout == 256 && !d.bias && !d.relu && !frag_epi;
+    const bool pair = pair_variant(kbn, d.deform != 0);
+    bool want_gn = false, gn_ok = tma_epi && d.Cout == 256 && !d.bias && !d.relu && !pair;
     for (int i = 0; i < nprob; ++i) {
         want_gn = want_gn || (probs[i].gn_stats != nullptr);
         if (pl.prob[i].BW * pl.prob[i].BH < 32) gn_ok = false;
@@ -1187,7 +1277,7 @@
     const int gn_fused = (want_gn && gn_ok) ? 1 : 0;
     const bool mem_bound = any_res || (d.KH * d.KW * (d.Cin / kBK) <= 8);
     int epi_bufs = mem_bound ? 2 : 1;
-    const int epi_merge = (d.split && tma_epi && !frag_epi && (mem_bound || d.stem == 2)) ? 1 : 0;
+    const int epi_merge = (d.split && tma_epi && !pair && (mem_bound || d.stem == 2)) ? 1 : 0;
     const int dcat = (d.split && d.deform) ? 1 : 0;
     const int ncat = (d.split && tma_epi && BN <= 128 && !d.deform && !any_res) ? 1 : 0;
     const int res_mma = (tma_epi && any_res) ? 1 : 0;
@@ -1208,7 +1298,7 @@
         int staging = d.out_f32 ? 0 : 128 * (hc * 2 + 16);
         if (tma_epi) staging = epi_bufs * (epi_merge ? 32768 : 16384);
         extra = (res_mma ? 8192 : 0) + (b_resident ? slab_bytes : 0) + staging;
-        stages = (kSmemPerBlock - (d.deform ? kStaticSmemDeform : kStaticSmemPlain) - dyn_smem_bytes(stage_b, 0, extra, frag_epi)) / stage_b;
+        stages = (kSmemPerBlock - (d.deform ? kStaticSmemDeform : kStaticSmemPlain) - dyn_smem_bytes(stage_b, 0, extra, pair)) / stage_b;
         if (stages >= 3) break;
         if (epi_bufs == 2) { epi_bufs = 1; continue; }
         if (b_resident) { b_resident = 0; continue; }
@@ -1217,6 +1307,18 @@
     }
     if (stages > kStagesMax) stages = kStagesMax;
     if (d.deform && stages > 3) stages = 3;
+    const bool frag = tma_epi && frag_epilogue(kbn, d.deform != 0);
+    const int region = frag ? region_slots(pair, epi_merge, gn_fused) : 0;
+    int epi_out = epi_bufs;
+    if (tma_epi && !d.deform) {
+        const int slot = epi_merge ? 32768 : 16384;
+        const int left = (kSmemPerBlock - kStaticSmemPlain - dyn_smem_bytes(stage_b, stages, extra, pair)) / slot;
+        const int spare = left < 4 - epi_bufs - region ? left : 4 - epi_bufs - region;
+        if (spare > 0) {
+            epi_out += spare;
+            extra += spare * slot;
+        }
+    }
 
     pl.num_m_tiles = mt;
     pl.kbn = kbn;
@@ -1233,6 +1335,9 @@
     }
     r.tma_epi = tma_epi; r.ncat = ncat; r.dcat = dcat; r.res_mma = res_mma; r.b_resident = b_resident;
     r.epi_merge = epi_merge; r.epi_bufs = epi_bufs; r.gn_fused = gn_fused; r.n_pair = n_pair;
+    r.frag_epi = frag ? 1 : 0;
+    r.epi_slots = tma_epi ? epi_out + region : 0;
+    pl.epi_out = epi_out;
     return ORP_OK;
 }
 
@@ -1265,6 +1370,7 @@
     P.ks_stride = (long long)P.prob[0].N * P.prob[0].Ho * P.prob[0].Wo * d.Cout;
     P.tma_epi = pl.rep.tma_epi; P.epi_bufs = pl.rep.epi_bufs; P.epi_merge = pl.rep.epi_merge; P.ncat = pl.rep.ncat;
     P.b_resident = pl.rep.b_resident; P.res_mma = pl.rep.res_mma; P.gn_fused = pl.rep.gn_fused; P.dcat = pl.rep.dcat;
+    P.epi_slots = pl.rep.epi_slots; P.epi_out = pl.epi_out;
     return ORP_OK;
 }
 
@@ -1349,7 +1455,7 @@
 int launch_tc(const TcParams &P, int stages, int grid, cudaStream_t st, int extra_bytes)
 {
     constexpr bool kCat = WALK == kWalkNcat || WALK == kWalkDcat;
-    const int smem = dyn_smem_bytes(stage_bytes(BN, kCat, P.b_resident), stages, extra_bytes, frag_epilogue(BN, DEFORM));
+    const int smem = dyn_smem_bytes(stage_bytes(BN, kCat, P.b_resident), stages, extra_bytes, pair_variant(BN, DEFORM));
     auto kern = conv_tc_kernel<BN, OUT_F32, DEFORM, SPLIT, WALK>;
     static int smem_max = -1;
     if (smem_max < 0) {
@@ -1405,7 +1511,7 @@
 {
     if constexpr (DEFORM) {
         if (P.dcat != P.split || P.ncat || P.res_mma) return fail(ORP_EINVAL, "conv2d_tc: deformable plan outside dcat == split");
-        if constexpr (frag_epilogue(BN, true)) {
+        if constexpr (pair_variant(BN, true)) {
             if (!P.split || OUT_F32 || !P.tma_epi || P.epi_merge || P.gn_fused || P.relu == 2)
                 return fail(ORP_EINVAL, "conv2d_tc: deformable N-tile pair outside f16x3 with an unmerged TMA epilogue and no GELU");
             return launch_tc<BN, false, true, true, kWalkDcat>(P, stages, grid, st, extra_bytes);
```

Measured after the change: 320.1, median of 6. Within noise of the previous version (-0.1%).
